# gopro/cineform-sdk

Hardware: AMD Instinct MI355X
Metric: 1080p YUY2 encode+decode fps (higher is better)
Workload: dtype int16

## Files before the change

cineform-sdk_amd/csrc/cfhd_entropy_gpu.h:

```cpp
#pragma once
#include "cfhd_core.h"
#include "cfhd_bitstream.h"
#include "cfhd_gop.h"
#include <vector>

namespace cfhd {

int device_stream_create(void **stream);
void device_stream_destroy(void *stream);
void device_stream_release(void *stream);
void device_streams_lean(bool on);
bool device_streams_are_lean();
struct StreamScope { StreamScope(); explicit StreamScope(void *preset ); ~StreamScope(); void *stream() const; };


class GpuEntropyEncoder {
public:
	GpuEntropyEncoder();
	~GpuEntropyEncoder();
	int prepare(const FramePlan &plan, int nframes, int16_t *d_coeffs, size_t coeff_stride_elems, size_t sample_cap, void *stream);
	int set_frame_header(int i, const SampleHeaderInfo &hdr);
	void set_plan(const FramePlan &plan) { plan_ = plan; }
	int prepare_group(const GopPlan &plan, int ngroups, int16_t *d_coeffs, size_t coeff_stride_elems, size_t sample_cap, void *stream);
	void set_group_plan(const GopPlan &plan) { gplan_ = plan; }
	int launch();
	int download();
	int download_queue();
	int download_finish();
	int fetch_sizes();
	const uint32_t *device_sizes() const { return d_sizes_; }
	const uint8_t *host_sample(int i) const { return h_samples_ + h_offsets_[i]; }
	uint8_t *device_sample(int i) { return d_samples_ + (size_t)i * cap_; }
	uint32_t sample_bytes(int i) const { return h_sizes_[i]; }
	void set_active(int k) { active_ = k; }
	void set_speculative_download(bool on) { speculative_download_ = on; if (!on) expect_bytes_ = 0; }
	bool needs_peak_table(int i) const { return peak_flags_in_use() && (h_sizes_[n_ + i] & 2u) != 0; }
	bool has_peak_table(int i) const { return peak_flags_in_use() && (h_sizes_[n_ + i] & 1u) != 0; }
	bool peak_flags_in_use() const { return group_ ? gplan_.interlaced : plan_.interlaced; }
	size_t sample_cap() const { return cap_; }
	int total_segments() const { return total_segs_; }
	float kernel_ms(int k);
	void set_level1_event(void *ev) { ev_level1_ = ev; }
	void *block_slots() const { return d_blocks_; }
	unsigned long long *block_masks(int frame) const { return d_masks_ ? d_masks_ + (size_t)frame * masks_per_frame_ : nullptr; }
	void set_block_lists(bool on) { use_blocks_ = on && d_blocks_; }
	bool block_lists() const { return use_blocks_; }
	void *headers_event() const { return ev_[3]; }
	void *samples_event() const { return ev_[4]; }
private:
	struct Host; Host *host_;
	void release();
	int prepare_units(int n, int16_t *d_coeffs, size_t coeff_stride_elems, size_t sample_cap, void *stream);
	void build_template(const SampleHeaderInfo &hdr, SampleTemplate *t) const;
	bool group_ = false; GopPlan gplan_;
	FramePlan plan_; int n_ = 0, active_ = 0, device_ = 0 ; size_t cap_ = 0; void *stream_ = nullptr;
	int active_frames() const { return active_ > 0 && active_ < n_ ? active_ : n_; }
	int nbands_ = 0, total_segs_ = 0;
	std::vector<SampleTemplate> tmpl_;
	uint8_t *d_samples_ = nullptr, *h_samples_ = nullptr;
	uint32_t *d_sizes_ = nullptr, *h_sizes_ = nullptr;
	uint8_t *d_packed_ = nullptr; uint32_t *d_offsets_ = nullptr, *h_offsets_ = nullptr;
	size_t expect_bytes_ = 0, copied_ahead_ = 0; int expect_frames_ = 0; bool speculative_download_ = false;
	void *d_tables_ = nullptr, *d_bands_ = nullptr, *d_segband_ = nullptr, *d_segs_ = nullptr, *d_bandstate_ = nullptr, *d_frames_ = nullptr, *d_tokens_ = nullptr;
	uint8_t *d_tmpl_ = nullptr, *h_tmpl_ = nullptr;
	bool dirty_ = true;
	void *ev_[5] = {nullptr, nullptr, nullptr, nullptr, nullptr}; bool timed_ = false;
	bool split_ = false, serial_split_ = false; void *ev_level1_ = nullptr, *stream2_ = nullptr, *ev2_[3] = {nullptr, nullptr, nullptr};
	int16_t *d_coeffs_ = nullptr; size_t coeff_stride_ = 0;
	void *d_blocks_ = nullptr; unsigned long long *d_masks_ = nullptr; size_t masks_per_frame_ = 0; bool use_blocks_ = false;
};


class GpuEntropyDecoder {
public:
	GpuEntropyDecoder();
	~GpuEntropyDecoder();
	void set_interlaced(bool on) { interlaced_ = on; }
	void set_active(int k) { active_ = k; }
	void set_skip_level1(bool skip) { skip_level1_ = skip; }
	int prepare(const FramePlan &plan, int nframes, int16_t *d_coeffs, size_t coeff_stride_elems, size_t sample_cap, int out_pixel_kind, void *stream);
	int set_sample_host(int i, const uint8_t *sample, size_t size);
	int set_sample_device(int i, const uint8_t *d_sample, const uint8_t *host_copy, size_t size);
	int set_samples_device(const uint8_t *d_samples, size_t stride_bytes, const uint32_t *d_sizes);
	void set_producer_events(void *headers, void *payloads) { ev_headers_ = headers; ev_payloads_ = payloads; }
	int launch();
	int check();
	float kernel_ms(int k);
	bool chunk_indexed() const { return dx_; }
	void *levels23_event() const { return l23_split_ ? ev_l23_ : nullptr; }
	void set_block_lists(bool on) { use_blocks_ = on && d_masks_; }
	bool level1_as_block_lists() const { return blocks_written_; }
	void dense_pyramid_uploaded() { blocks_written_ = false; }
	const unsigned long long *block_masks(int frame) const { return d_masks_ ? d_masks_ + (size_t)frame * masks_per_frame_ : nullptr; }
	int stats(uint32_t out[16]);
private:
	struct Host; Host *host_;
	void release();
	FramePlan plan_; int n_ = 0, out_kind_ = 0; size_t cap_ = 0, coeff_stride_ = 0; void *stream_ = nullptr;
	int16_t *d_coeffs_ = nullptr;
	uint8_t *d_samples_ = nullptr, *h_samples_ = nullptr;
	void *d_tables_ = nullptr, *d_bandjobs_ = nullptr, *d_lowjobs_ = nullptr, *d_plan_ = nullptr;
	void *ev_headers_ = nullptr, *ev_payloads_ = nullptr;
	bool skip_level1_ = false, interlaced_ = false; void *d_diffjobs_ = nullptr;
	int active_ = 0;
	int active_frames() const { return active_ > 0 && active_ < n_ ? active_ : n_; }
	const uint8_t *ext_samples_ = nullptr; size_t ext_stride_ = 0; const uint32_t *ext_sizes_ = nullptr;
	int *d_errors_ = nullptr, *h_errors_ = nullptr;
	bool lane_kernel_ = false;
	bool dx_ = true;
	void *d_tile_start_ = nullptr, *d_stats_ = nullptr, *d_repair_ = nullptr, *d_alts_ = nullptr, *d_reindex_ = nullptr, *d_alt_entries_ = nullptr; uint32_t alt_slots_ = 0;
	void *d_idx_tables_ = nullptr, *d_entries_ = nullptr, *d_recs_ = nullptr, *d_chunk_base_ = nullptr, *d_chunk_job_ = nullptr, *d_sums_ = nullptr, *d_counters_ = nullptr;
	uint32_t max_chunks_ = 0, *h_counters_ = nullptr; void *h_chunk_job_ = nullptr;
	int grid_index_ = 0, grid_tiles_ = 0;
	int device_ = 0;
	int launch_dx(bool device_jobs, int njobs, uint32_t host_chunks, int lowpass_jobs);
	void *ev_l23_ = nullptr, *ev_low_ = nullptr; bool l23_split_ = false;
	void *ev_[8] = {nullptr, nullptr, nullptr, nullptr, nullptr, nullptr, nullptr, nullptr}; bool timed_ = false;
	bool parse_end_ = false;
	unsigned long long *d_masks_ = nullptr; size_t masks_per_frame_ = 0; bool use_blocks_ = false, blocks_written_ = false;
};

class GpuGroupEntropyDecoder {
public:
	GpuGroupEntropyDecoder() {}
	~GpuGroupEntropyDecoder() { release(); }
	int prepare(const GopPlan &plan, int16_t *d_coeffs, size_t sample_cap, int out_pixel_kind, void *stream, int device = -1);
	int launch(const uint8_t *sample, size_t size, const ParsedGroup &pg);
	int check();
	void release();
private:
	GopPlan plan_; int out_kind_ = 0, device_ = 0; size_t cap_ = 0; void *stream_ = nullptr;
	int16_t *d_coeffs_ = nullptr;
	uint8_t *d_sample_ = nullptr, *h_sample_ = nullptr;
	void *d_tables_ = nullptr, *d_bandjobs_ = nullptr, *d_lowjobs_ = nullptr, *h_bandjobs_ = nullptr, *h_lowjobs_ = nullptr;
	void *d_tables18_ = nullptr, *d_diffjobs_ = nullptr, *h_diffjobs_ = nullptr;
	int *d_errors_ = nullptr, *h_errors_ = nullptr;
};

}
```

cineform-sdk_amd/csrc/cfhd_entropy_gpu.hip:

```cpp
#include "cfhd_entropy_gpu.h"
#include "cfhd_entropy_jobs.h"
#include <hip/hip_runtime.h>
#include <string.h>
#include <stdio.h>
#include <stdlib.h>
#include <algorithm>

namespace cfhd {

int device_init();
int device_current();
namespace { int g_fail(hipError_t e, const char *what) { fprintf(stderr, "[cfhd_amd] %s: %s\n", what, hipGetErrorString(e)); return (int)e ? (int)e : -1; } }
#define HIPCHK(expr) do { hipError_t _e = (expr); if (_e != hipSuccess) return g_fail(_e, #expr); } while (0)

struct GpuEntropyEncoder::Host { EntHostJobs jobs; std::vector<EntHoleGeom> geom; dev::EntFrameJob *frames = nullptr;  };

GpuEntropyEncoder::GpuEntropyEncoder() : host_(new Host) {}
GpuEntropyEncoder::~GpuEntropyEncoder() { release(); delete host_; }

void GpuEntropyEncoder::release()
{
	(void)hipSetDevice(device_);
	void *dev[] = { d_samples_, d_sizes_, d_tables_, d_bands_, d_segband_, d_segs_, d_bandstate_, d_frames_, d_tmpl_, d_packed_, d_offsets_, d_tokens_, d_blocks_, d_masks_ };
	for (void *p : dev) if (p) (void)hipFree(p);
	if (h_samples_) (void)hipHostFree(h_samples_);
	if (h_sizes_) (void)hipHostFree(h_sizes_);
	if (h_offsets_) (void)hipHostFree(h_offsets_);
	d_packed_ = nullptr; d_offsets_ = h_offsets_ = nullptr;
	if (h_tmpl_) (void)hipHostFree(h_tmpl_);
	if (host_->frames) { (void)hipHostFree(host_->frames); host_->frames = nullptr; }
	for (void *&e : ev_) if (e) { (void)hipEventDestroy((hipEvent_t)e); e = nullptr; }
	for (void *&e : ev2_) if (e) { (void)hipEventDestroy((hipEvent_t)e); e = nullptr; }
	if (stream2_) { device_stream_destroy(stream2_); stream2_ = nullptr; }
	timed_ = false;
	d_samples_ = h_samples_ = nullptr; d_sizes_ = h_sizes_ = nullptr; d_tables_ = d_bands_ = d_segband_ = d_segs_ = d_bandstate_ = d_frames_ = d_tokens_ = nullptr;
	d_tmpl_ = h_tmpl_ = nullptr; n_ = 0;
	d_blocks_ = nullptr; d_masks_ = nullptr; masks_per_frame_ = 0; use_blocks_ = false;
}

int GpuEntropyEncoder::prepare(const FramePlan &plan, int nframes, int16_t *d_coeffs, size_t stride, size_t sample_cap, void *stream)
{
	group_ = false; plan_ = plan;
	return prepare_units(nframes, d_coeffs, stride, sample_cap, stream);
}

int GpuEntropyEncoder::prepare_group(const GopPlan &plan, int ngroups, int16_t *d_coeffs, size_t stride, size_t sample_cap, void *stream)
{
	group_ = true; gplan_ = plan; plan_ = FramePlan(); plan_.interlaced = false;
	return prepare_units(ngroups, d_coeffs, stride, sample_cap, stream);
}

void GpuEntropyEncoder::build_template(const SampleHeaderInfo &hdr, SampleTemplate *t) const
{
	if (group_) build_group_template(gplan_, hdr, t); else build_sample_template(plan_, hdr, t);
}

int GpuEntropyEncoder::prepare_units(int nframes, int16_t *d_coeffs, size_t stride, size_t sample_cap, void *stream)
{
	int rc = device_init();
	if (rc) return rc;
	release();
	device_ = device_current(); (void)hipSetDevice(device_);
	const FramePlan &plan = plan_;
	n_ = nframes; cap_ = (sample_cap + 255) & ~(size_t)255; stream_ = stream; d_coeffs_ = d_coeffs; coeff_stride_ = stride;
	if (cap_ * (size_t)n_ >= ((size_t)1 << 32)) { fprintf(stderr, "[cfhd_amd] batch of %d frames exceeds the 4 GiB sample arena\n", n_); return -5; }
	{
		std::vector<dev::EntTables> h(2);
		ent_build_tables(&h[0], 1); ent_build_tables(&h[1], 2);
		HIPCHK(hipMalloc(&d_tables_, 2 * sizeof(dev::EntTables)));
		HIPCHK(hipMemcpy(d_tables_, h.data(), 2 * sizeof(dev::EntTables), hipMemcpyHostToDevice));
	}
	SampleHeaderInfo hdr0 = { 1, 2, 2, 4, !plan.interlaced, nullptr, 0, nullptr, 0 };
	tmpl_.assign(n_, SampleTemplate());
	build_template(hdr0, &tmpl_[0]);
	EntHostJobs &jobs = host_->jobs;
	host_->geom = group_ ? ent_hole_geometry(gplan_, tmpl_[0]) : ent_hole_geometry(plan, tmpl_[0]);
	if (!ent_build_band_jobs(host_->geom, tmpl_[0], n_, d_coeffs, stride, &jobs)) return -3;
	nbands_ = jobs.nbands; total_segs_ = (int)jobs.segjobs.size();
	HIPCHK(hipMalloc(&d_bands_, jobs.bands.size() * sizeof(dev::EntBandJob)));
	HIPCHK(hipMemcpy(d_bands_, jobs.bands.data(), jobs.bands.size() * sizeof(dev::EntBandJob), hipMemcpyHostToDevice));
	HIPCHK(hipMalloc(&d_segband_, jobs.segjobs.size() * sizeof(dev::EntSegJob)));
	HIPCHK(hipMemcpy(d_segband_, jobs.segjobs.data(), jobs.segjobs.size() * sizeof(dev::EntSegJob), hipMemcpyHostToDevice));
	HIPCHK(hipMalloc(&d_segs_, jobs.segjobs.size() * sizeof(dev::EntSegState)));
	HIPCHK(hipMalloc(&d_tokens_, jobs.segjobs.size() * (size_t)dev::ENT_TOK_STRIDE * sizeof(uint32_t)));
	HIPCHK(hipMalloc(&d_bandstate_, jobs.bands.size() * sizeof(dev::EntBandState)));
	static_assert((int)kBlockChunkCols == (int)dev::FWD_CHUNK_COLS_ENT, "one chunk geometry");
	if (!group_ && !plan.interlaced && plan.encoded_format == ENC_YUV422 && (plan.pixel_kind == PIX_YUY2 || plan.pixel_kind == PIX_2VUY) && plan.width % 32 == 0) {
		int mask_base[kMaxChannels][kNumBands];
		masks_per_frame_ = (size_t)block_list_layout(plan, mask_base);
		HIPCHK(hipMalloc(&d_blocks_, stride * 2 * (size_t)n_));
		HIPCHK(hipMalloc((void **)&d_masks_, masks_per_frame_ * 8 * (size_t)n_ + 64));
		HIPCHK(hipMemset(d_masks_, 0, masks_per_frame_ * 8 * (size_t)n_ + 64));
	}
	HIPCHK(hipMalloc((void **)&d_samples_, cap_ * n_));
	HIPCHK(hipHostMalloc((void **)&h_samples_, cap_ * n_, hipHostMallocPortable));
	HIPCHK(hipMalloc((void **)&d_sizes_, sizeof(uint32_t) * 2 * n_));
	HIPCHK(hipHostMalloc((void **)&h_sizes_, sizeof(uint32_t) * 2 * n_, hipHostMallocPortable));
	memset(h_sizes_, 0, sizeof(uint32_t) * 2 * n_);
	HIPCHK(hipMalloc((void **)&d_packed_, cap_ * n_));
	HIPCHK(hipMalloc((void **)&d_offsets_, sizeof(uint32_t) * (n_ + 1)));
	HIPCHK(hipHostMalloc((void **)&h_offsets_, sizeof(uint32_t) * (n_ + 1), hipHostMallocPortable));
	memset(h_offsets_, 0, sizeof(uint32_t) * (n_ + 1));
	HIPCHK(hipMalloc((void **)&d_tmpl_, (size_t)kEntTmplStride * n_));
	HIPCHK(hipHostMalloc((void **)&h_tmpl_, (size_t)kEntTmplStride * n_, hipHostMallocPortable));
	memset(h_tmpl_, 0, (size_t)kEntTmplStride * n_);
	HIPCHK(hipMalloc(&d_frames_, n_ * sizeof(dev::EntFrameJob)));
	HIPCHK(hipHostMalloc((void **)&host_->frames, n_ * sizeof(dev::EntFrameJob), hipHostMallocPortable));
	for (int f = 0; f < n_; f++) { SampleHeaderInfo h = hdr0; h.frame_number = (uint32_t)f + 1; if ((rc = set_frame_header(f, h))) return rc; }
	for (void *&e : ev_) HIPCHK(hipEventCreate((hipEvent_t *)&e));
	for (void *&e : ev2_) HIPCHK(hipEventCreate((hipEvent_t *)&e));
	if (n_ >= 8 || !device_streams_are_lean()) HIPCHK((hipError_t)device_stream_create(&stream2_));
	return 0;
}

int GpuEntropyEncoder::set_frame_header(int f, const SampleHeaderInfo &hdr)
{
	if (f < 0 || f >= n_) return -1;
	SampleTemplate &t = tmpl_[f];
	build_template(hdr, &t);
	if (!ent_fill_frame_block(host_->geom, t, f, host_->jobs, d_coeffs_ + (size_t)f * coeff_stride_, h_tmpl_ + (size_t)kEntTmplStride * f)) return -4;
	host_->frames[f] = ent_frame_job(t, d_tmpl_ + (size_t)kEntTmplStride * f, d_samples_ + cap_ * f, (uint32_t)cap_, d_sizes_ + f, d_sizes_ + n_ + f);
	dirty_ = true;
	return 0;
}

int GpuEntropyEncoder::launch()
{
	(void)hipSetDevice(device_);
	hipStream_t st = (hipStream_t)stream_;
	if (dirty_) {
		HIPCHK(hipMemcpyAsync(d_tmpl_, h_tmpl_, (size_t)kEntTmplStride * n_, hipMemcpyHostToDevice, st));
		HIPCHK(hipMemcpyAsync(d_frames_, host_->frames, n_ * sizeof(dev::EntFrameJob), hipMemcpyHostToDevice, st));
		dirty_ = false;
	}
	const dev::EntTables *T = (const dev::EntTables *)d_tables_;
	const dev::EntBatchGeom geom = { total_segs_ / n_, nbands_, coeff_stride_ };
	const int act = active_frames(), total_segs = total_segs_ / n_ * act;
	(void)hipGetLastError();
	HIPCHK(hipEventRecord((hipEvent_t)ev_[0], st));
#ifdef CFHD_AMD_PROBES
	const int count_probe = []{ const char *e = getenv("CFHD_AMD_COUNT_PROBE"); return e ? atoi(e) : 0; }();
#else
	const int count_probe = 0;
#endif
	const dev::EntBlockLists lists = { (const uint4 *)d_blocks_, d_masks_, d_coeffs_, masks_per_frame_ };
	auto count_range = [&](hipStream_t s, int lo, int n, bool level1 = false) {
		const int total = n * act;
		if (level1 && use_blocks_)
			dev::k_ent_count_blocks<<<(total + dev::ENT_WAVES - 1) / dev::ENT_WAVES, dev::ENT_THREADS, 0, s>>>((const dev::EntSegJob *)d_segband_, geom, total, (dev::EntSegState *)d_segs_, T,
			                                                                                                 d_sizes_ + n_, (uint32_t *)d_tokens_, lo, n, lists);
		else
			dev::k_ent_count<<<(total + dev::ENT_WAVES - 1) / dev::ENT_WAVES, dev::ENT_THREADS, 0, s>>>((const dev::EntSegJob *)d_segband_, geom, total, (dev::EntSegState *)d_segs_, T,
			                                                                                          d_sizes_ + n_, (uint32_t *)d_tokens_, lo, n, count_probe);
	};
	static const bool split_on = [] { const char *e = getenv("CFHD_AMD_COUNT_SPLIT"); return !(e && atoi(e) == 0); }();
	split_ = split_on && ev_level1_ && stream2_ && !host_->jobs.ranges_l1.empty() && act >= 8;
	if (peak_flags_in_use() && !split_) HIPCHK(hipMemsetAsync(d_sizes_ + n_, 0, sizeof(uint32_t) * n_, st));
	serial_split_ = split_ && stream2_ == stream_;
	if (serial_split_) {
		if (peak_flags_in_use()) HIPCHK(hipMemsetAsync(d_sizes_ + n_, 0, sizeof(uint32_t) * n_, st));
		HIPCHK(hipEventRecord((hipEvent_t)ev2_[0], st));
		for (const auto &r : host_->jobs.ranges_l1) count_range(st, r.first, r.second, true);
		HIPCHK(hipEventRecord((hipEvent_t)ev2_[1], st));
		for (const auto &r : host_->jobs.ranges_rest) count_range(st, r.first, r.second);
		HIPCHK(hipEventRecord((hipEvent_t)ev2_[2], st));
	} else if (split_) {
		hipStream_t s2 = (hipStream_t)stream2_;
		HIPCHK(hipStreamWaitEvent(s2, (hipEvent_t)ev_level1_, 0));
		if (peak_flags_in_use()) HIPCHK(hipMemsetAsync(d_sizes_ + n_, 0, sizeof(uint32_t) * n_, s2));
		HIPCHK(hipEventRecord((hipEvent_t)ev2_[0], s2));
		for (const auto &r : host_->jobs.ranges_l1) count_range(s2, r.first, r.second, true);
		HIPCHK(hipEventRecord((hipEvent_t)ev2_[1], s2));
		for (const auto &r : host_->jobs.ranges_rest) count_range(st, r.first, r.second);
		HIPCHK(hipEventRecord((hipEvent_t)ev2_[2], st));
		HIPCHK(hipStreamWaitEvent(st, (hipEvent_t)ev2_[1], 0));
	} else if (use_blocks_) {
		for (const auto &r : host_->jobs.ranges_l1) count_range(st, r.first, r.second, true);
		for (const auto &r : host_->jobs.ranges_rest) count_range(st, r.first, r.second);
	} else count_range(st, 0, total_segs_ / n_);
	HIPCHK(hipEventRecord((hipEvent_t)ev_[1], st));
	dev::k_ent_scan<<<nbands_ * act, dev::ENT_THREADS, 0, st>>>((const dev::EntBandJob *)d_bands_, (dev::EntSegState *)d_segs_, (dev::EntBandState *)d_bandstate_, T);
	HIPCHK(hipEventRecord((hipEvent_t)ev_[2], st));
	const unsigned layout_parts = act >= 256 ? 8u : (unsigned)((2048 + act - 1) / act > 256 ? 256 : (2048 + act - 1) / act);
	dev::k_ent_layout<<<dim3((unsigned)act, layout_parts), dev::ENT_THREADS, 0, st>>>((const dev::EntFrameJob *)d_frames_, (const dev::EntBandJob *)d_bands_, (dev::EntSegState *)d_segs_,
	                                                  (dev::EntBandState *)d_bandstate_, T);
	HIPCHK(hipEventRecord((hipEvent_t)ev_[3], st));
	{
		dev::EntPeakHoles which; which.n = 0;
		for (size_t h = 0; h < tmpl_[0].holes.size() && which.n < 7; h++) if (tmpl_[0].holes[h].kind == 2) which.hole[which.n++] = (int)h;
		if (which.n) dev::k_ent_peaks<<<dim3(act >= 64 ? 4u : 32u, (unsigned)which.n, (unsigned)act), dev::ENT_THREADS, 0, st>>>((const dev::EntFrameJob *)d_frames_, which, (const dev::EntBandJob *)d_bands_,
		                                                  (const dev::EntSegJob *)d_segband_, geom, (const dev::EntSegState *)d_segs_, (const dev::EntBandState *)d_bandstate_);
	}
#ifdef CFHD_AMD_PROBES
	const int emit_probe = []{ const char *e = getenv("CFHD_AMD_EMIT_PROBE"); return e ? atoi(e) : 0; }();
#else
	const int emit_probe = 0;
#endif
	dev::k_ent_emit<<<(total_segs + dev::ENT_WAVES * dev::ENT_EMIT_SEGS - 1) / (dev::ENT_WAVES * dev::ENT_EMIT_SEGS), dev::ENT_THREADS, 0, st>>>(total_segs, (const dev::EntSegState *)d_segs_,
	                                                          T, (const uint32_t *)d_tokens_, emit_probe);
	HIPCHK(hipGetLastError());
	HIPCHK(hipEventRecord((hipEvent_t)ev_[4], st));
	timed_ = true;
	return 0;
}

float GpuEntropyEncoder::kernel_ms(int k)
{
	float ms = 0;
	if (!timed_ || k < 0 || k > 4) return 0;
	if (k == 4) {
		if (!split_ || hipEventElapsedTime(&ms, (hipEvent_t)ev2_[0], (hipEvent_t)ev2_[1]) != hipSuccess) { (void)hipGetLastError(); return 0; }
		return ms;
	}
	void *end = (k == 0 && split_) ? ev2_[2] : ev_[k + 1];
	void *begin = (k == 0 && serial_split_) ? ev2_[1] : ev_[k];
	if (hipEventElapsedTime(&ms, (hipEvent_t)begin, (hipEvent_t)end) != hipSuccess) { (void)hipGetLastError(); return 0; }
	return ms;
}

int GpuEntropyEncoder::fetch_sizes()
{
	(void)hipSetDevice(device_);
	hipStream_t st = (hipStream_t)stream_;
	HIPCHK(hipMemcpyAsync(h_sizes_, d_sizes_, sizeof(uint32_t) * 2 * n_, hipMemcpyDeviceToHost, st));
	HIPCHK(hipStreamSynchronize(st));
	return 0;
}

int GpuEntropyEncoder::download() { const int rc = download_queue(); return rc ? rc : download_finish(); }

int GpuEntropyEncoder::download_queue()
{
	(void)hipSetDevice(device_);
	hipStream_t st = (hipStream_t)stream_;
	const bool direct = false;
	(void)hipGetLastError();
	const int act = active_frames();
	dev::k_ent_pack_offsets<<<1, dev::ENT_THREADS, 0, st>>>(d_sizes_, act, d_offsets_);
	dev::k_ent_pack<<<dim3(direct ? 2 : 8, (unsigned)act), dev::ENT_THREADS, 0, st>>>(d_samples_, cap_, d_sizes_, d_offsets_, direct ? h_samples_ : d_packed_);
	HIPCHK(hipGetLastError());
	HIPCHK(hipMemcpyAsync(h_sizes_, d_sizes_, sizeof(uint32_t) * 2 * n_, hipMemcpyDeviceToHost, st));
	HIPCHK(hipMemcpyAsync(h_offsets_, d_offsets_, sizeof(uint32_t) * (act + 1), hipMemcpyDeviceToHost, st));
	copied_ahead_ = 0;
	if (!direct && expect_bytes_ && expect_frames_ == act) {
		copied_ahead_ = expect_bytes_ < cap_ * (size_t)act ? expect_bytes_ : cap_ * (size_t)act;
		HIPCHK(hipMemcpyAsync(h_samples_, d_packed_, copied_ahead_, hipMemcpyDeviceToHost, st));
	}
	return 0;
}

int GpuEntropyEncoder::download_finish()
{
	(void)hipSetDevice(device_);
	hipStream_t st = (hipStream_t)stream_;
	const bool direct = false;
	const int act = active_frames();
	HIPCHK(hipStreamSynchronize(st));
	const size_t total = h_offsets_[act];
	if (!direct && total > copied_ahead_) HIPCHK(hipMemcpyAsync(h_samples_ + copied_ahead_, d_packed_ + copied_ahead_, total - copied_ahead_, hipMemcpyDeviceToHost, st));
	expect_bytes_ = speculative_download_ ? ((total + total / 32 + 4095) & ~(size_t)4095) : 0; expect_frames_ = act;
	return 0;
}

struct GpuEntropyDecoder::Host {
	std::vector<std::vector<dev::DecBandJob>> bands;
	std::vector<std::vector<dev::DecLowpassJob>> lows;
	std::vector<size_t> host_bytes;
	std::vector<std::vector<dev::DecDiffJob>> diffs;
	dev::DecBandJob *flat_bands = nullptr; dev::DecLowpassJob *flat_lows = nullptr; dev::DecDiffJob *flat_diffs = nullptr;
};

GpuEntropyDecoder::GpuEntropyDecoder() : host_(new Host) {}
GpuEntropyDecoder::~GpuEntropyDecoder() { release(); delete host_; }

void GpuEntropyDecoder::release()
{
	(void)hipSetDevice(device_);
	void *dev[] = { d_samples_, d_tables_, d_bandjobs_, d_lowjobs_, d_errors_, d_plan_, d_idx_tables_, d_entries_, d_recs_, d_chunk_base_, d_chunk_job_, d_sums_, d_counters_, d_tile_start_, d_stats_, d_repair_, d_alts_, d_reindex_, d_diffjobs_, d_alt_entries_, d_masks_ };
	d_masks_ = nullptr; masks_per_frame_ = 0; use_blocks_ = false; blocks_written_ = false;
	for (void *p : dev) if (p) (void)hipFree(p);
	d_idx_tables_ = d_entries_ = d_recs_ = d_chunk_base_ = d_chunk_job_ = d_sums_ = d_counters_ = d_tile_start_ = d_stats_ = d_repair_ = d_alts_ = d_reindex_ = d_diffjobs_ = d_alt_entries_ = nullptr;
	if (h_chunk_job_) (void)hipHostFree(h_chunk_job_);
	if (h_counters_) (void)hipHostFree(h_counters_);
	h_chunk_job_ = nullptr; h_counters_ = nullptr;
	if (h_samples_) (void)hipHostFree(h_samples_);
	if (h_errors_) (void)hipHostFree(h_errors_);
	if (host_->flat_bands) { (void)hipHostFree(host_->flat_bands); host_->flat_bands = nullptr; }
	if (host_->flat_lows) { (void)hipHostFree(host_->flat_lows); host_->flat_lows = nullptr; }
	if (host_->flat_diffs) { (void)hipHostFree(host_->flat_diffs); host_->flat_diffs = nullptr; }
	for (void *&e : ev_) if (e) { (void)hipEventDestroy((hipEvent_t)e); e = nullptr; }
	if (ev_l23_) { (void)hipEventDestroy((hipEvent_t)ev_l23_); ev_l23_ = nullptr; }
	if (ev_low_) { (void)hipEventDestroy((hipEvent_t)ev_low_); ev_low_ = nullptr; }
	timed_ = false;
	d_samples_ = h_samples_ = nullptr; d_tables_ = d_bandjobs_ = d_lowjobs_ = d_plan_ = nullptr; d_errors_ = h_errors_ = nullptr; n_ = 0; ext_samples_ = nullptr;
}

int GpuEntropyDecoder::prepare(const FramePlan &plan, int nframes, int16_t *d_coeffs, size_t stride, size_t sample_cap, int out_kind, void *stream)
{
	int rc = device_init();
	if (rc) return rc;
	release();
	device_ = device_current(); (void)hipSetDevice(device_);
	plan_ = plan; n_ = nframes; cap_ = (sample_cap + 255) & ~(size_t)255; stream_ = stream; d_coeffs_ = d_coeffs; coeff_stride_ = stride; out_kind_ = out_kind;
	std::vector<uint32_t> t = build_dec_tables(1);
	HIPCHK(hipMalloc(&d_tables_, t.size() * 4));
	HIPCHK(hipMemcpy(d_tables_, t.data(), t.size() * 4, hipMemcpyHostToDevice));
	HIPCHK(hipMalloc((void **)&d_samples_, cap_ * n_));
	HIPCHK(hipHostMalloc((void **)&h_samples_, cap_ * n_, hipHostMallocPortable));
	const size_t max_bands = (size_t)n_ * kMaxChannels * 9, max_lows = (size_t)n_ * kMaxChannels;
	HIPCHK(hipMalloc(&d_bandjobs_, max_bands * sizeof(dev::DecBandJob)));
	HIPCHK(hipMalloc(&d_lowjobs_, max_lows * sizeof(dev::DecLowpassJob)));
	HIPCHK(hipHostMalloc((void **)&host_->flat_bands, max_bands * sizeof(dev::DecBandJob), hipHostMallocPortable));
	HIPCHK(hipHostMalloc((void **)&host_->flat_lows, max_lows * sizeof(dev::DecLowpassJob), hipHostMallocPortable));
	HIPCHK(hipMalloc(&d_diffjobs_, max_lows * sizeof(dev::DecDiffJob)));
	HIPCHK(hipHostMalloc((void **)&host_->flat_diffs, max_lows * sizeof(dev::DecDiffJob), hipHostMallocPortable));
	HIPCHK(hipMalloc((void **)&d_errors_, sizeof(int)));
	HIPCHK(hipHostMalloc((void **)&h_errors_, sizeof(int), hipHostMallocPortable));
	*h_errors_ = 0;
	{ const char *e = getenv("CFHD_AMD_DEC"); lane_kernel_ = e && strcmp(e, "lane") == 0; dx_ = !(e && (strcmp(e, "lane") == 0 || strcmp(e, "par") == 0)); }
	if (dx_) {
		dev::DecIdxTables *it = new dev::DecIdxTables;
		const bool ok = build_dec_index_tables(1, it);
		if (ok) { hipError_t e = hipMalloc(&d_idx_tables_, sizeof(*it)); if (e == hipSuccess) e = hipMemcpy(d_idx_tables_, it, sizeof(*it), hipMemcpyHostToDevice); if (e != hipSuccess) { delete it; return g_fail(e, "decoder tables"); } }
		delete it;
		if (!ok) return -6;
		const size_t per_frame = cap_ / dev::DX_CHUNK_BYTES + (size_t)kMaxChannels * 9 + 1;
		if (per_frame * (size_t)n_ >= ((size_t)1 << 31) / dev::DX_ENTRY_STRIDE * 8) return -5;
		max_chunks_ = (uint32_t)(per_frame * (size_t)n_);
		HIPCHK(hipMalloc(&d_entries_, (size_t)max_chunks_ * dev::DX_ENTRY_STRIDE * 4));
		HIPCHK(hipMalloc(&d_recs_, (size_t)max_chunks_ * sizeof(dev::DxChunkRec)));
		HIPCHK(hipMalloc(&d_chunk_base_, (size_t)max_chunks_ * 4));
		HIPCHK(hipMalloc(&d_chunk_job_, (size_t)max_chunks_ * sizeof(dev::DxChunkDesc)));
		HIPCHK(hipMalloc(&d_sums_, max_bands * sizeof(dev::DxBandSum)));
		HIPCHK(hipMalloc(&d_counters_, 32));
		HIPCHK(hipMalloc(&d_repair_, max_bands * 4));
		HIPCHK(hipMalloc(&d_alts_, (size_t)max_chunks_ * sizeof(dev::DxChunkAlt)));
		HIPCHK(hipMalloc(&d_reindex_, (size_t)max_chunks_ * sizeof(dev::DxReindex)));
		alt_slots_ = max_chunks_ / 8 > 64u ? max_chunks_ / 8 : 64u;
		HIPCHK(hipMalloc(&d_alt_entries_, (size_t)alt_slots_ * dev::DX_ENTRY_STRIDE * 4));
		{
			dev::DecPlan dp0; dec_build_plan(plan, out_kind, &dp0);
			const dev::DxTilePlan tp0 = dx_tile_plan(plan, dp0, n_, false);
			HIPCHK(hipMalloc(&d_tile_start_, ((size_t)tp0.total + 1) * sizeof(dev::DxTileDesc)));
			const char *se = getenv("CFHD_AMD_DX_STATS");
			if (se && atoi(se)) { HIPCHK(hipMalloc(&d_stats_, 64)); HIPCHK(hipMemset(d_stats_, 0, 64)); }
		}
		HIPCHK(hipHostMalloc((void **)&h_chunk_job_, (size_t)max_chunks_ * sizeof(dev::DxChunkDesc), hipHostMallocPortable));
		HIPCHK(hipHostMalloc((void **)&h_counters_, 32, hipHostMallocPortable));
		int cus = 256;
		(void)hipDeviceGetAttribute(&cus, hipDeviceAttributeMultiprocessorCount, device_current());
		grid_index_ = cus * 5; grid_tiles_ = cus * (int)((160 * 1024) / (sizeof(uint2) * (1 << dev::DX_KM) + sizeof(uint32_t) * (dev::DX_LONG11_MAX + dev::DX_TILE_WORDS)));
		if (const char *e = getenv("CFHD_AMD_DX_GRID_TILES")) if (atoi(e) > 0) grid_tiles_ = atoi(e);
		if (grid_index_ < 1) grid_index_ = 1;
		if (grid_tiles_ < 1) grid_tiles_ = 1;
	}
	{
		dev::DecPlan dp;
		dec_build_plan(plan, out_kind, &dp);
		HIPCHK(hipMalloc(&d_plan_, sizeof(dp)));
		HIPCHK(hipMemcpy(d_plan_, &dp, sizeof(dp), hipMemcpyHostToDevice));
	}
	if (dx_ && plan.encoded_format == ENC_YUV422 && plan.num_channels == 3) {
		int mask_base[kMaxChannels][kNumBands];
		masks_per_frame_ = (size_t)dec_block_list_layout(plan, mask_base);
		HIPCHK(hipMalloc((void **)&d_masks_, masks_per_frame_ * 8 * (size_t)n_));
	}
	host_->bands.assign(n_, {}); host_->lows.assign(n_, {}); host_->diffs.assign(n_, {}); host_->host_bytes.assign(n_, 0);
	for (void *&e : ev_) HIPCHK(hipEventCreate((hipEvent_t *)&e));
	HIPCHK(hipEventCreate((hipEvent_t *)&ev_l23_));
	HIPCHK(hipEventCreate((hipEvent_t *)&ev_low_));
	return 0;
}

int GpuEntropyDecoder::set_samples_device(const uint8_t *d_samples, size_t stride_bytes, const uint32_t *d_sizes)
{
	if (!d_samples || !d_sizes || (stride_bytes & 255) || ((uintptr_t)d_samples & 255)) return -1;
	ext_samples_ = d_samples; ext_stride_ = stride_bytes; ext_sizes_ = d_sizes;
	return 0;
}

int GpuEntropyDecoder::set_sample_host(int i, const uint8_t *sample, size_t size)
{
	if (i < 0 || i >= n_ || size > cap_) return -1;
	memcpy(h_samples_ + cap_ * i, sample, size);
	int rc = set_sample_device(i, d_samples_ + cap_ * i, sample, size);
	if (rc == 0) host_->host_bytes[i] = (size + 3) & ~(size_t)3;
	return rc;
}

int GpuEntropyDecoder::set_sample_device(int i, const uint8_t *d_sample, const uint8_t *host_copy, size_t size)
{
	if (i < 0 || i >= n_) return -1;
	ext_samples_ = nullptr;
	ParsedSample ps;
	if (parse_sample(host_copy, size, &ps) != 0) return -2;
	if (ps.width != plan_.width || ps.display_height != plan_.display_height || ps.encoded_format != plan_.encoded_format || ps.num_channels != plan_.num_channels) return -3;
	host_->bands[i].clear(); host_->lows[i].clear(); host_->host_bytes[i] = 0;
	if (dx_) {
		dev::DecPlan dp; dec_build_plan(plan_, out_kind_, &dp);
		host_->bands[i].assign((size_t)dp.bands_per_frame, dev::DecBandJob());
		host_->lows[i].assign((size_t)plan_.num_channels, dev::DecLowpassJob());
		host_->diffs[i].assign((size_t)plan_.num_channels, dev::DecDiffJob());
		if (!dx_build_jobs(ps, plan_, dp, d_sample, d_coeffs_ + (size_t)i * coeff_stride_, out_kind_, 0, 1, host_->bands[i].data(), host_->lows[i].data(), skip_level1_,
		                   interlaced_ ? host_->diffs[i].data() : nullptr)) return -4;
		return 0;
	}
	if (interlaced_) return -4;
	if (!dec_build_jobs(ps, plan_, d_sample, d_coeffs_ + (size_t)i * coeff_stride_, out_kind_, &host_->bands[i], &host_->lows[i], skip_level1_)) return -4;
	return 0;
}

enum { kLowLatencyFrames = 32 };

int GpuEntropyDecoder::launch()
{
	(void)hipSetDevice(device_);
	hipStream_t st = (hipStream_t)stream_;
	l23_split_ = false; blocks_written_ = false;
	if (ext_samples_) {
		const int nch = plan_.num_channels, nb = n_ * nch * 9;
		HIPCHK(hipMemsetAsync(d_errors_, 0, sizeof(int), st));
		(void)hipGetLastError();
		static const bool parse_early = [] { const char *e = getenv("CFHD_AMD_PARSE_EARLY"); return !(e && atoi(e) == 0); }();
		if (!parse_early && ev_payloads_) ev_headers_ = ev_payloads_;
		if (ev_headers_) HIPCHK(hipStreamWaitEvent(st, (hipEvent_t)ev_headers_, 0));
		HIPCHK(hipEventRecord((hipEvent_t)ev_[0], st));
		dev::k_dec_parse<<<n_, dev::DEC_PARSE_THREADS, 0, st>>>(ext_samples_, ext_stride_, ext_sizes_, n_,
			(const dev::DecPlan *)d_plan_, d_coeffs_, coeff_stride_, (dev::DecBandJob *)d_bandjobs_, (dev::DecLowpassJob *)d_lowjobs_, d_errors_,
			interlaced_ && dx_ ? (dev::DecDiffJob *)d_diffjobs_ : nullptr);
		parse_end_ = ev_payloads_ != nullptr;
		if (parse_end_) { HIPCHK(hipEventRecord((hipEvent_t)ev_[4], st)); HIPCHK(hipStreamWaitEvent(st, (hipEvent_t)ev_payloads_, 0)); }
		ev_headers_ = ev_payloads_ = nullptr;
		HIPCHK(hipEventRecord((hipEvent_t)ev_[1], st));
		l23_split_ = false;
		if (dx_) { const int rc_dx = launch_dx(true, nb, 0u, n_ * nch); if (rc_dx) return rc_dx; }
		else if (n_ <= kLowLatencyFrames) dev::k_dec_bands_par_ll<<<nb, dev::DECP_LL_THREADS, 0, st>>>((const dev::DecBandJob *)d_bandjobs_, (const dev::DecTables *)d_tables_, d_errors_);
		else dev::k_dec_bands_par<<<nb, dev::DECP_THREADS, 0, st>>>((const dev::DecBandJob *)d_bandjobs_, (const dev::DecTables *)d_tables_, d_errors_);
		HIPCHK(hipEventRecord((hipEvent_t)ev_[2], st));
		if (!l23_split_) dev::k_dec_lowpass<<<dim3(8, (unsigned)(n_ * nch)), 256, 0, st>>>((const dev::DecLowpassJob *)d_lowjobs_);
		HIPCHK(hipGetLastError());
		HIPCHK(hipEventRecord((hipEvent_t)ev_[3], st));
		timed_ = true;
		HIPCHK(hipMemcpyAsync(h_errors_, d_errors_, sizeof(int), hipMemcpyDeviceToHost, st));
		return 0;
	}
	parse_end_ = false;
	if (dx_) {
		dev::DecPlan dp; dec_build_plan(plan_, out_kind_, &dp);
		const int nch = plan_.num_channels, act = active_frames(), nb = dp.bands_per_frame * act;
		HIPCHK(hipStreamSynchronize(st));
		for (int f = 0; f < act; f++) {
			if ((int)host_->bands[f].size() != dp.bands_per_frame || (int)host_->lows[f].size() != nch) return -1;
			for (int s = 0; s < dp.bands_per_frame; s++) host_->flat_bands[(size_t)s * act + f] = host_->bands[f][s];
			for (int c = 0; c < nch; c++) host_->flat_lows[(size_t)f * nch + c] = host_->lows[f][c];
			if (interlaced_) { if ((int)host_->diffs[f].size() != nch) return -1; for (int c = 0; c < nch; c++) host_->flat_diffs[(size_t)f * nch + c] = host_->diffs[f][c]; }
		}
		std::vector<dev::DxChunkDesc> cj;
		const uint32_t nchunks = dx_number_chunks(host_->flat_bands, nb, &cj);
		if (nchunks > max_chunks_) return -5;
		memcpy(h_chunk_job_, cj.data(), cj.size() * sizeof(dev::DxChunkDesc));
		h_counters_[0] = nchunks; h_counters_[1] = 0; h_counters_[2] = 0; h_counters_[3] = 0; h_counters_[4] = 0;
		HIPCHK(hipMemsetAsync(d_errors_, 0, sizeof(int), st));
		for (int f = 0; f < act; f++)
			if (host_->host_bytes[f]) HIPCHK(hipMemcpyAsync(d_samples_ + cap_ * f, h_samples_ + cap_ * f, host_->host_bytes[f], hipMemcpyHostToDevice, st));
		HIPCHK(hipMemcpyAsync(d_bandjobs_, host_->flat_bands, (size_t)nb * sizeof(dev::DecBandJob), hipMemcpyHostToDevice, st));
		HIPCHK(hipMemcpyAsync(d_lowjobs_, host_->flat_lows, (size_t)act * nch * sizeof(dev::DecLowpassJob), hipMemcpyHostToDevice, st));
		if (interlaced_) HIPCHK(hipMemcpyAsync(d_diffjobs_, host_->flat_diffs, (size_t)act * nch * sizeof(dev::DecDiffJob), hipMemcpyHostToDevice, st));
		HIPCHK(hipMemcpyAsync(d_chunk_job_, h_chunk_job_, (size_t)nchunks * sizeof(dev::DxChunkDesc), hipMemcpyHostToDevice, st));
		HIPCHK(hipMemcpyAsync(d_counters_, h_counters_, 20, hipMemcpyHostToDevice, st));
		(void)hipGetLastError();
		HIPCHK(hipEventRecord((hipEvent_t)ev_[0], st));
		HIPCHK(hipEventRecord((hipEvent_t)ev_[1], st));
		l23_split_ = false;
		int rc = launch_dx(false, nb, nchunks, act * nch);
		if (rc) return rc;
		HIPCHK(hipEventRecord((hipEvent_t)ev_[2], st));
		if (!l23_split_) dev::k_dec_lowpass<<<dim3(8, (unsigned)(act * nch)), 256, 0, st>>>((const dev::DecLowpassJob *)d_lowjobs_);
		HIPCHK(hipGetLastError());
		HIPCHK(hipEventRecord((hipEvent_t)ev_[3], st));
		timed_ = true;
		HIPCHK(hipMemcpyAsync(h_errors_, d_errors_, sizeof(int), hipMemcpyDeviceToHost, st));
		return 0;
	}
	const bool lane_kernel = lane_kernel_;
	dev::DecBandJob *fb = host_->flat_bands; dev::DecLowpassJob *fl = host_->flat_lows;
	size_t nfb = 0, nfl = 0, per_frame = 0;
	for (int f = 0; f < n_; f++) per_frame = host_->bands[f].size() > per_frame ? host_->bands[f].size() : per_frame;
	for (size_t k = 0; k < per_frame; k++) for (int f = 0; f < n_; f++) if (k < host_->bands[f].size()) fb[nfb++] = host_->bands[f][k];
	for (int f = 0; f < n_; f++) for (const dev::DecLowpassJob &j : host_->lows[f]) fl[nfl++] = j;
	if (!nfb) return -1;
	if (!lane_kernel) std::stable_sort(fb, fb + nfb, [](const dev::DecBandJob &a, const dev::DecBandJob &b) { return a.bytes > b.bytes; });
	else HIPCHK(hipMemset2DAsync(d_coeffs_, coeff_stride_ * 2, 0, (size_t)plan_.final_elems * 2, n_, st));
	HIPCHK(hipMemsetAsync(d_errors_, 0, sizeof(int), st));
	for (int f = 0; f < n_; f++)
		if (host_->host_bytes[f]) HIPCHK(hipMemcpyAsync(d_samples_ + cap_ * f, h_samples_ + cap_ * f, host_->host_bytes[f], hipMemcpyHostToDevice, st));
	HIPCHK(hipMemcpyAsync(d_bandjobs_, fb, nfb * sizeof(dev::DecBandJob), hipMemcpyHostToDevice, st));
	HIPCHK(hipMemcpyAsync(d_lowjobs_, fl, nfl * sizeof(dev::DecLowpassJob), hipMemcpyHostToDevice, st));
	(void)hipGetLastError();
	const int nb = (int)nfb;
	HIPCHK(hipEventRecord((hipEvent_t)ev_[0], st));
	HIPCHK(hipEventRecord((hipEvent_t)ev_[1], st));
	if (lane_kernel) dev::k_dec_bands<<<(nb + dev::DEC_THREADS - 1) / dev::DEC_THREADS, dev::DEC_THREADS, 0, st>>>((const dev::DecBandJob *)d_bandjobs_, nb, (const dev::DecTables *)d_tables_, d_errors_);
	else if (n_ <= kLowLatencyFrames) dev::k_dec_bands_par_ll<<<nb, dev::DECP_LL_THREADS, 0, st>>>((const dev::DecBandJob *)d_bandjobs_, (const dev::DecTables *)d_tables_, d_errors_);
	else dev::k_dec_bands_par<<<nb, dev::DECP_THREADS, 0, st>>>((const dev::DecBandJob *)d_bandjobs_, (const dev::DecTables *)d_tables_, d_errors_);
	HIPCHK(hipEventRecord((hipEvent_t)ev_[2], st));
	dev::k_dec_lowpass<<<dim3(8, (unsigned)nfl), 256, 0, st>>>((const dev::DecLowpassJob *)d_lowjobs_);
	HIPCHK(hipGetLastError());
	HIPCHK(hipEventRecord((hipEvent_t)ev_[3], st));
	timed_ = true;
	HIPCHK(hipMemcpyAsync(h_errors_, d_errors_, sizeof(int), hipMemcpyDeviceToHost, st));
	return 0;
}

int GpuEntropyDecoder::launch_dx(bool device_jobs, int njobs, uint32_t host_chunks, int lowpass_jobs)
{
	hipStream_t st = (hipStream_t)stream_;
	dev::DecBandJob *jobs = (dev::DecBandJob *)d_bandjobs_;
	const dev::DecIdxTables *T = (const dev::DecIdxTables *)d_idx_tables_;
	dev::DecPlan dp; dec_build_plan(plan_, out_kind_, &dp);
	const int frames = device_jobs ? n_ : active_frames();
	const bool lists = use_blocks_ && d_masks_ && !skip_level1_;
	const dev::DxTilePlan tp = dx_tile_plan(plan_, dp, frames, skip_level1_, lists, interlaced_);
	unsigned long long *const tmasks = lists ? d_masks_ : nullptr;
	blocks_written_ = lists;
	const char *spec_env = getenv("CFHD_AMD_DX_SPECULATE");
	const bool speculate = !(spec_env && atoi(spec_env) == 0);
	if (device_jobs) HIPCHK(hipMemsetAsync((uint32_t *)d_counters_ + 1, 0, 16, st));
	if (device_jobs) {
		dev::k_dec_plan<<<1, 1024, 0, st>>>(jobs, njobs, max_chunks_, (uint32_t *)d_counters_, d_errors_);
		dev::k_dec_plan_fill<<<(njobs + dev::DX_WAVES - 1) / dev::DX_WAVES, dev::DX_THREADS, 0, st>>>(jobs, njobs, (dev::DxChunkDesc *)d_chunk_job_, (const uint32_t *)d_counters_);
	}
	HIPCHK(hipEventRecord((hipEvent_t)ev_[7], st));
	const uint32_t chunk_bound = device_jobs ? max_chunks_ : host_chunks;
	int g1 = grid_index_, g3 = grid_tiles_;
	if ((uint32_t)g1 * dev::DX_WAVES > chunk_bound) g1 = (int)((chunk_bound + dev::DX_WAVES - 1) / dev::DX_WAVES);
	const uint32_t tile_waves = 1u;
	if ((uint32_t)g3 > tp.total) g3 = (int)tp.total;
	if (g1 < 1) g1 = 1;
	if (g3 < 1) g3 = 1;
	dev::k_dec_index<<<g1, dev::DX_THREADS, 0, st>>>((const dev::DxChunkDesc *)d_chunk_job_, (const uint32_t *)d_counters_, T, (uint32_t *)d_entries_, (dev::DxChunkRec *)d_recs_, (dev::DxChunkAlt *)d_alts_, speculate ? 1 : 0, (uint32_t *)d_stats_,
	                                                 (uint32_t *)d_alt_entries_, alt_slots_, (uint32_t *)d_counters_ + 3, (uint32_t *)d_counters_ + 4);
	HIPCHK(hipEventRecord((hipEvent_t)ev_[5], st));
	dev::k_dec_chain<<<(njobs + dev::DX_WAVES - 1) / dev::DX_WAVES, dev::DX_THREADS, 0, st>>>(jobs, njobs, (const dev::DxChunkRec *)d_recs_, (const dev::DxChunkAlt *)d_alts_, (uint32_t *)d_chunk_base_,
	                                                                                            (dev::DxBandSum *)d_sums_, d_errors_, (uint32_t *)d_repair_, (dev::DxReindex *)d_reindex_, (uint32_t *)d_counters_);
	const int small_grid = njobs < 256 ? (njobs + dev::DX_WAVES - 1) / dev::DX_WAVES : 64;
	dev::k_dec_repair<<<small_grid, dev::DX_THREADS, 0, st>>>(jobs, T, (uint32_t *)d_entries_, (dev::DxChunkRec *)d_recs_, (const dev::DxChunkAlt *)d_alts_, (uint32_t *)d_chunk_base_, (dev::DxBandSum *)d_sums_,
	                                                         d_errors_, (const uint32_t *)d_repair_, (dev::DxReindex *)d_reindex_, (uint32_t *)d_counters_, (uint32_t *)d_stats_);
	dev::k_dec_reindex<<<g1, dev::DX_THREADS, 0, st>>>(jobs, T, (uint32_t *)d_entries_, (const dev::DxReindex *)d_reindex_, (const uint32_t *)d_counters_, (uint32_t *)d_stats_,
	                                                   (const dev::DxChunkAlt *)d_alts_, (const uint32_t *)d_alt_entries_);
	dev::k_dec_tile_index<<<(tp.total + dev::DX_TILE_INDEX_TILES - 1) / dev::DX_TILE_INDEX_TILES, dev::DX_THREADS, 0, st>>>(jobs, tp, (const uint32_t *)d_entries_, (const uint32_t *)d_chunk_base_, (const dev::DxBandSum *)d_sums_,
	                                                                                                  (dev::DxTileDesc *)d_tile_start_, tmasks, (uint32_t)masks_per_frame_);
	HIPCHK(hipEventRecord((hipEvent_t)ev_[6], st));
	const char *split_env = getenv("CFHD_AMD_TILES_SPLIT");
	l23_split_ = frames >= 8 && !skip_level1_ && tp.split > 0 && tp.split < tp.total && split_env && split_env[0] == '1';
	auto tile_pass = [&](const dev::DxTilePlan &p, int g) {
		dev::k_dec_tiles<dev::DX_TILE_THREADS><<<g < 1 ? 1 : g, dev::DX_TILE_THREADS, 0, st>>>((const dev::DxTileDesc *)d_tile_start_, p.first, p.total, T, (const uint32_t *)d_entries_, (const uint32_t *)d_chunk_base_);
	};
	if (l23_split_) {
		dev::DxTilePlan ta = tp, tb = tp;
		ta.total = tp.split; tb.first = tp.split;
		int ga = g3, gb = g3;
		if ((uint32_t)ga * tile_waves > ta.total) ga = (int)((ta.total + tile_waves - 1) / tile_waves);
		if ((uint32_t)gb * tile_waves > tb.total - tb.first) gb = (int)((tb.total - tb.first + tile_waves - 1) / tile_waves);
		tile_pass(ta, ga);
		HIPCHK(hipEventRecord((hipEvent_t)ev_low_, st));
		dev::k_dec_lowpass<<<dim3(8, (unsigned)lowpass_jobs), 256, 0, st>>>((const dev::DecLowpassJob *)d_lowjobs_);
		HIPCHK(hipEventRecord((hipEvent_t)ev_l23_, st));
		tile_pass(tb, gb);
	} else tile_pass(tp, g3);
	if (interlaced_) {
		const bool rows = true;
		if (rows) dev::k_dec_undiff_rows<<<dim3((unsigned)(frames * plan_.num_channels), 32), 64 * dev::DXR_WAVES, 0, st>>>((const dev::DecDiffJob *)d_diffjobs_);
		dev::k_dec_undiff<<<dim3((unsigned)(frames * plan_.num_channels), dev::DXU_SPLIT), dev::DXU_THREADS, 0, st>>>((const dev::DecDiffJob *)d_diffjobs_, d_errors_, rows ? 1 : 0);
	}
	HIPCHK(hipGetLastError());
	return 0;
}

int GpuEntropyDecoder::check() { return *h_errors_ ? -1 : 0; }

int GpuEntropyDecoder::stats(uint32_t out[16])
{
	(void)hipSetDevice(device_);
	memset(out, 0, 64);
	if (!d_stats_) return -1;
	HIPCHK(hipStreamSynchronize((hipStream_t)stream_));
	HIPCHK(hipMemcpy(out, d_stats_, 64, hipMemcpyDeviceToHost));
	return 0;
}

float GpuEntropyDecoder::kernel_ms(int k)
{
	float ms = 0;
	if (k >= 3) {
		if (!timed_ || !dx_ || k > 6) return 0;
		void *a = k == 3 ? ev_[7] : (k == 4 ? ev_[5] : (k == 5 ? ev_[6] : ev_[1])), *b = k == 3 ? ev_[5] : (k == 4 ? ev_[6] : (k == 5 ? ev_[2] : ev_[7]));
		if (hipEventElapsedTime(&ms, (hipEvent_t)a, (hipEvent_t)b) != hipSuccess) { (void)hipGetLastError(); return 0; }
		if (k == 5 && l23_split_) {
			float low = 0;
			if (hipEventElapsedTime(&low, (hipEvent_t)ev_low_, (hipEvent_t)ev_l23_) == hipSuccess) ms -= low; else (void)hipGetLastError();
		}
		return ms;
	}
	if (k == 2 && l23_split_ && timed_) {
		if (hipEventElapsedTime(&ms, (hipEvent_t)ev_low_, (hipEvent_t)ev_l23_) != hipSuccess) { (void)hipGetLastError(); return 0; }
		return ms;
	}
	void *end = (k == 0 && parse_end_) ? ev_[4] : ev_[k + 1];
	if (!timed_ || k < 0 || k > 2 || hipEventElapsedTime(&ms, (hipEvent_t)ev_[k], (hipEvent_t)end) != hipSuccess) { (void)hipGetLastError(); return 0; }
	return ms;
}

void GpuGroupEntropyDecoder::release()
{
	(void)hipSetDevice(device_);
	void *dev[] = { d_sample_, d_tables_, d_tables18_, d_bandjobs_, d_lowjobs_, d_diffjobs_, d_errors_ };
	for (void *p : dev) if (p) (void)hipFree(p);
	void *host[] = { h_sample_, h_bandjobs_, h_lowjobs_, h_diffjobs_, h_errors_ };
	for (void *p : host) if (p) (void)hipHostFree(p);
	d_sample_ = h_sample_ = nullptr; d_tables_ = d_tables18_ = d_bandjobs_ = d_lowjobs_ = d_diffjobs_ = h_bandjobs_ = h_lowjobs_ = h_diffjobs_ = nullptr; d_errors_ = h_errors_ = nullptr;
}

enum { kGroupBandJobs = 3 * 15, kGroupRawJobs = 3 * 2, kGroupDiffJobs = 3 * 2 };

int GpuGroupEntropyDecoder::prepare(const GopPlan &plan, int16_t *d_coeffs, size_t sample_cap, int out_kind, void *stream, int device)
{
	int rc = device_init();
	if (rc) return rc;
	release();
	device_ = device >= 0 ? device : device_current(); (void)hipSetDevice(device_);
	plan_ = plan; d_coeffs_ = d_coeffs; cap_ = (sample_cap + 255) & ~(size_t)255; out_kind_ = out_kind; stream_ = stream;
	std::vector<uint32_t> t = build_dec_tables(1);
	HIPCHK(hipMalloc(&d_tables_, t.size() * 4));
	HIPCHK(hipMemcpy(d_tables_, t.data(), t.size() * 4, hipMemcpyHostToDevice));
	t = build_dec_tables(2);
	HIPCHK(hipMalloc(&d_tables18_, t.size() * 4));
	HIPCHK(hipMemcpy(d_tables18_, t.data(), t.size() * 4, hipMemcpyHostToDevice));
	HIPCHK(hipMalloc(&d_diffjobs_, kGroupDiffJobs * sizeof(dev::DecDiffJob)));
	HIPCHK(hipHostMalloc(&h_diffjobs_, kGroupDiffJobs * sizeof(dev::DecDiffJob), hipHostMallocPortable));
	HIPCHK(hipMalloc((void **)&d_sample_, cap_));
	HIPCHK(hipHostMalloc((void **)&h_sample_, cap_, hipHostMallocPortable));
	HIPCHK(hipMalloc(&d_bandjobs_, kGroupBandJobs * sizeof(dev::DecBandJob)));
	HIPCHK(hipMalloc(&d_lowjobs_, kGroupRawJobs * sizeof(dev::DecLowpassJob)));
	HIPCHK(hipHostMalloc(&h_bandjobs_, kGroupBandJobs * sizeof(dev::DecBandJob), hipHostMallocPortable));
	HIPCHK(hipHostMalloc(&h_lowjobs_, kGroupRawJobs * sizeof(dev::DecLowpassJob), hipHostMallocPortable));
	HIPCHK(hipMalloc((void **)&d_errors_, sizeof(int)));
	HIPCHK(hipHostMalloc((void **)&h_errors_, sizeof(int), hipHostMallocPortable));
	*h_errors_ = 0;
	return 0;
}

int GpuGroupEntropyDecoder::launch(const uint8_t *sample, size_t size, const ParsedGroup &pg)
{
	(void)hipSetDevice(device_);
	hipStream_t st = (hipStream_t)stream_;
	if (size > cap_) return -1;
	HIPCHK(hipStreamSynchronize(st));
	dev::DecBandJob *bj = (dev::DecBandJob *)h_bandjobs_; dev::DecLowpassJob *lj = (dev::DecLowpassJob *)h_lowjobs_; dev::DecDiffJob *dj = (dev::DecDiffJob *)h_diffjobs_;
	int nb = 0, nl = 0, nd = 0;
	for (int c = 0; c < 3; c++) {
		const GopChannel &ch = plan_.ch[c];
		const ParsedBand &lp = pg.lowpass[c];
		const GopWavelet &top = ch.w[5];
		if (!lp.present || lp.width != top.width || lp.height != top.height || (size_t)lp.offset + (size_t)top.width * top.height * 2 > size) return -2;
		lj[nl++] = dev::DecLowpassJob{ d_sample_ + lp.offset, d_coeffs_ + top.offset[0], top.width, top.height, top.pitch, 2 * lowpass_bias(10, top.width, out_kind_) };
		static const int coded[5] = { 5, 4, 3, 1, 0 };
		for (int k : coded) {
			const GopWavelet &wv = ch.w[k];
			for (int b = (k == 3 ? 0 : 1); b < 4; b++) {
				const ParsedBand &pb = pg.band[c][k][b];
				if (!pb.present || pb.width != wv.width || pb.height != wv.height || (pb.offset & 3) || (size_t)pb.offset + pb.bytes > size) return -2;
				if (pb.codebook < 0) {
					if ((size_t)pb.bytes < (size_t)wv.width * wv.height * 2 || pb.quant != 1 || (wv.width & 1)) return -3;
					lj[nl++] = dev::DecLowpassJob{ d_sample_ + pb.offset, d_coeffs_ + wv.offset[0], wv.width, wv.height, wv.pitch, 0 };
					continue;
				}
				const bool diff = gop_band_is_difference_coded(plan_, k, b);
				if (pb.codebook != (diff ? 2 : 1) || pb.difference != diff || (wv.offset[b] & 7) || (wv.pitch & 7)) return -3;
				if (diff) {
					if (nd >= kGroupDiffJobs || wv.width > 16 * 256 || (pb.peak_level && (size_t)pb.peak_offset + 2 > size)) return -3;
					dj[nd++] = dev::DecDiffJob{ d_coeffs_ + wv.offset[b], wv.width, wv.height, wv.pitch, pb.peak_level ? d_sample_ + pb.peak_offset : nullptr,
					                            pb.peak_level ? (uint32_t)(size - pb.peak_offset) : 0u, pb.peak_level };
				}
				bj[nb++] = dev::DecBandJob{ d_sample_ + pb.offset, pb.bytes, d_coeffs_ + wv.offset[b], wv.height * wv.pitch, pb.quant, 0u, diff ? 1 : 0 };
			}
		}
	}
	if (nb != kGroupBandJobs || nl != kGroupRawJobs || nd != (plan_.interlaced ? kGroupDiffJobs : 0)) return -2;
	std::stable_sort(bj, bj + nb, [](const dev::DecBandJob &a, const dev::DecBandJob &b) { return a.table != b.table ? a.table < b.table : a.bytes > b.bytes; });
	const int nb18 = nd, nb17 = nb - nb18;
	memcpy(h_sample_, sample, size);
	HIPCHK(hipMemsetAsync(d_errors_, 0, sizeof(int), st));
	HIPCHK(hipMemcpyAsync(d_sample_, h_sample_, (size + 3) & ~(size_t)3, hipMemcpyHostToDevice, st));
	HIPCHK(hipMemcpyAsync(d_bandjobs_, bj, nb * sizeof(dev::DecBandJob), hipMemcpyHostToDevice, st));
	HIPCHK(hipMemcpyAsync(d_lowjobs_, lj, nl * sizeof(dev::DecLowpassJob), hipMemcpyHostToDevice, st));
	(void)hipGetLastError();
	dev::k_dec_bands_par_ll<<<nb17, dev::DECP_LL_THREADS, 0, st>>>((const dev::DecBandJob *)d_bandjobs_, (const dev::DecTables *)d_tables_, d_errors_);
	if (nb18) {
		HIPCHK(hipMemcpyAsync(d_diffjobs_, dj, nd * sizeof(dev::DecDiffJob), hipMemcpyHostToDevice, st));
		dev::k_dec_bands_par_ll<<<nb18, dev::DECP_LL_THREADS, 0, st>>>((const dev::DecBandJob *)d_bandjobs_ + nb17, (const dev::DecTables *)d_tables18_, d_errors_);
		dev::k_dec_undiff<<<dim3((unsigned)nd, dev::DXU_SPLIT), dev::DXU_THREADS, 0, st>>>((const dev::DecDiffJob *)d_diffjobs_, d_errors_, 0);
	}
	dev::k_dec_lowpass<<<dim3(8, (unsigned)nl), 256, 0, st>>>((const dev::DecLowpassJob *)d_lowjobs_);
	HIPCHK(hipGetLastError());
	HIPCHK(hipMemcpyAsync(h_errors_, d_errors_, sizeof(int), hipMemcpyDeviceToHost, st));
	return 0;
}

int GpuGroupEntropyDecoder::check() { return h_errors_ ? *h_errors_ : -1; }

}
```

cineform-sdk_amd/csrc/cfhd_entropy_jobs.h:

```cpp
#pragma once
#include "cfhd_core.h"
#include "cfhd_bitstream.h"
#include "cfhd_gop.h"
#include "cfhd_entropy_kernels.h"
#include "cfhd_dec_kernels.h"
#include <vector>
#include <algorithm>
#include <string.h>

namespace cfhd {

enum { kEntTmplBytes = 6144, kEntWordHolesBytes = 1536, kEntHolesBytes = dev::ENT_MAX_HOLES * (int)sizeof(dev::EntHole), kEntMaxPatches = 96,
       kEntPatchBytes = kEntMaxPatches * (int)sizeof(dev::EntPatch), kEntTmplStride = kEntTmplBytes + kEntWordHolesBytes + kEntHolesBytes + kEntPatchBytes };

inline void ent_build_tables(dev::EntTables *h, int codebook = 1)
{
	const EntropyTables *t = entropy_tables(codebook);
	memcpy(h->value_code, t->value_code, sizeof(h->value_code));
	memcpy(h->run_bits, t->run_bits, sizeof(h->run_bits));
	for (int c = 0; c < 3072; c++) { h->run_count[c] = t->run_count[c]; h->run_size[c] = t->run_size[c]; }
	h->run_total[0] = 0;
	for (int c = 1; c < 3072; c++) h->run_total[c] = (uint16_t)(t->run_size[c] + h->run_total[c - t->run_count[c]]);
	h->band_end_bits = t->band_end_bits; h->band_end_size = t->band_end_size;
	for (int c = 0; c < 3072; c++) { h->run_pack[c].x = t->run_bits[c]; h->run_pack[c].y = (uint32_t)t->run_size[c] | ((uint32_t)t->run_count[c] << 8); }
}

std::vector<uint32_t> build_dec_tables(int codebook);

inline bool build_dec_index_tables(int codebook, dev::DecIdxTables *T)
{
	using namespace dev;
	memset(T, 0, sizeof(*T));
	RawCode codes[300];
	const int ncodes = raw_codes(codebook, codes);
	const EntropyTables *et = entropy_tables(codebook);
	for (int m = 0; m < 256; m++) { T->mag_expand[0][m] = entropy_tables(1)->mag_expand[m]; T->mag_expand[1][m] = entropy_tables(2)->mag_expand[m]; }
	(void)et;
	auto type_of = [](const RawCode &c) { return c.kind == 0 ? DX_T_RUN : (c.kind == 1 ? DX_T_VALUE : DX_T_END); };
	uint32_t nlong = 0;
	int l2_of_prefix[1 << DX_K];
	for (int p = 0; p < (1 << DX_K); p++) l2_of_prefix[p] = -1;
	for (int i = 0; i < ncodes; i++) {
		const RawCode &c = codes[i];
		if (c.len <= DX_K) {
			if (c.kind == 2 || c.payload >= (1 << 11) || c.len > 12) return false;
			const uint32_t base = c.bits << (DX_K - c.len);
			const uint16_t e = (uint16_t)(c.len | (c.kind == 1 ? 16 : 0) | (c.payload << 5));
			for (uint32_t k = 0; k < (1u << (DX_K - c.len)); k++) T->sym12[base + k] = e;
		} else {
			if (c.len > DX_K + 2 * DX_L2_BITS) return false;
			const uint32_t p = c.bits >> (c.len - DX_K);
			if (l2_of_prefix[p] < 0) {
				if (nlong + (1u << DX_L2_BITS) > DX_LONG_MAX || nlong >= (1u << 11)) return false;
				l2_of_prefix[p] = (int)nlong; nlong += 1u << DX_L2_BITS;
				T->sym12[p] = (uint16_t)(16u | ((uint32_t)l2_of_prefix[p] << 5));
			}
		}
	}
	struct L3 { uint32_t key; int maxlen; uint32_t base; };
	std::vector<L3> l3;
	for (int i = 0; i < ncodes; i++) {
		const RawCode &c = codes[i];
		if (c.len <= DX_K + DX_L2_BITS) continue;
		const uint32_t key = c.bits >> (c.len - DX_K - DX_L2_BITS);
		auto it = std::find_if(l3.begin(), l3.end(), [&](const L3 &x) { return x.key == key; });
		if (it == l3.end()) l3.push_back(L3{ key, c.len, 0 }); else if (c.len > it->maxlen) it->maxlen = c.len;
	}
	for (L3 &x : l3) {
		const int nb = x.maxlen - DX_K - DX_L2_BITS;
		if (nlong + (1u << nb) > DX_LONG_MAX) return false;
		x.base = nlong; nlong += 1u << nb;
		const uint32_t p = x.key >> DX_L2_BITS;
		T->long_tab[(uint32_t)l2_of_prefix[p] + (x.key & ((1u << DX_L2_BITS) - 1u))] = (uint32_t)nb | ((uint32_t)DX_T_ESCAPE << 5) | (x.base << 8);
	}
	for (int i = 0; i < ncodes; i++) {
		const RawCode &c = codes[i];
		if (c.len <= DX_K) continue;
		const uint32_t entry = (c.kind == 2 ? 0u : (uint32_t)c.len + (c.kind == 1 ? 1u : 0u)) | ((uint32_t)type_of(c) << 5) | ((c.kind == 0 ? (uint32_t)c.payload : (c.kind == 1 ? 1u : 0u)) << 8);
		if (c.len <= DX_K + DX_L2_BITS) {
			const uint32_t p = c.bits >> (c.len - DX_K);
			const int spare = DX_K + DX_L2_BITS - c.len;
			const uint32_t base = (uint32_t)l2_of_prefix[p] + ((c.bits & ((1u << (c.len - DX_K)) - 1u)) << spare);
			for (uint32_t k = 0; k < (1u << spare); k++) T->long_tab[base + k] = entry;
		} else {
			const uint32_t key = c.bits >> (c.len - DX_K - DX_L2_BITS);
			const L3 &x = *std::find_if(l3.begin(), l3.end(), [&](const L3 &y) { return y.key == key; });
			const int nb = x.maxlen - DX_K - DX_L2_BITS, rest = c.len - DX_K - DX_L2_BITS, spare = nb - rest;
			const uint32_t base = x.base + ((c.bits & ((1u << rest) - 1u)) << spare);
			for (uint32_t k = 0; k < (1u << spare); k++) T->long_tab[base + k] = entry;
		}
	}
	T->nlong = nlong;
	for (uint32_t win = 0; win < (1u << DX_K); win++) {
		int used = 0; uint32_t count = 0;
		for (;;) {
			const uint32_t rest = (win << used) & ((1u << DX_K) - 1u);
			const uint16_t e = T->sym12[rest];
			const int len = e & 15, total = len + ((e & 16) ? 1 : 0);
			if (!len || total > DX_K - used) break;
			const uint32_t add = (e & 16) ? 1u : (uint32_t)(e >> 5);
			if (count + add > 4095u) break;
			used += total; count += add;
		}
		T->cnt12[win] = (uint16_t)(used | (count << 4));
	}
	for (uint32_t win = 0; win < (1u << DX_KM); win++) {
		int used = 0, pre = 0, mid = 0, post = 0, v1 = 0, v2 = 0;
		for (;;) {
			const uint32_t rest = ((win << (DX_K - DX_KM)) << used) & ((1u << DX_K) - 1u);
			const uint16_t e = T->sym12[rest];
			const int len = e & 15, total = len + ((e & 16) ? 1 : 0);
			if (!len || total > DX_KM - used) break;
			if (e & 16) {
				if (v2) break;
				const int m = e >> 5;
				if (T->mag_expand[0][m] != m || T->mag_expand[1][m] != m || m > 0x7fff) return false;
				const int negative = (int)((rest >> (DX_K - len - 1)) & 1u);
				if (!v1) v1 = negative ? -m : m; else v2 = negative ? -m : m;
			} else {
				const int run = e >> 5;
				int *slot = v2 ? &post : (v1 ? &mid : &pre);
				if (*slot + run > (slot == &pre ? 0xfff : 0xff)) break;
				*slot += run;
			}
			used += total;
		}
		if (v1 && !v2) { post = mid; mid = 0; }
		const int total = pre + (v1 ? 1 : 0) + mid + (v2 ? 1 : 0) + post;
		const uint32_t o1 = v1 ? (uint32_t)pre : (uint32_t)DX_NO_VALUE, o2 = v2 ? (uint32_t)(pre + 1 + mid) : (uint32_t)DX_NO_VALUE;
		if (total > 0xfff || v1 < -128 || v1 > 127 || v2 < -128 || v2 > 127 || (v1 && pre >= (int)DX_NO_VALUE) || (v2 && pre + 1 + mid >= (int)DX_NO_VALUE)) return false;
		T->multi[win].x = (uint32_t)(used & 15) | ((uint32_t)total << 4) | (o1 << 16);
		T->multi[win].y = o2 | ((uint32_t)(uint8_t)(int8_t)v1 << 16) | ((uint32_t)(uint8_t)(int8_t)v2 << 24);
	}
	{
		auto entry_of = [&](const RawCode &c, bool *ok) {
			const uint32_t a = c.kind == 1 ? T->mag_expand[0][c.payload] : (c.kind == 0 ? (uint32_t)c.payload : 0u), b = c.kind == 1 ? T->mag_expand[1][c.payload] : a;
			const uint32_t bits = (uint32_t)c.len + (c.kind == 1 ? 1u : 0u);
			if (a >= (1u << 12) || b >= (1u << 12) || bits > 31u) *ok = false;
			return bits | ((uint32_t)type_of(c) << 5) | (a << 8) | (b << 20);
		};
		bool ok = true;
		uint32_t n11 = 0;
		int l2_of[1 << DX_KM];
		for (int p = 0; p < (1 << DX_KM); p++) l2_of[p] = -1;
		struct L3b { uint32_t key; int maxlen; uint32_t base; };
		std::vector<L3b> l3b;
		for (int i = 0; i < ncodes; i++) {
			const RawCode &c = codes[i];
			const int total = c.len + (c.kind == 1 ? 1 : 0);
			if (total <= DX_KM) continue;
			if (c.len <= DX_KM) {
				const uint32_t base = c.bits << (DX_KM - c.len);
				for (uint32_t k = 0; k < (1u << (DX_KM - c.len)); k++) { if (T->multi[base + k].x & 15u) ok = false; T->multi[base + k].y = entry_of(c, &ok); }
				continue;
			}
			const uint32_t p11 = c.bits >> (c.len - DX_KM);
			if (l2_of[p11] < 0) {
				if (n11 + (1u << DX_L11_BITS) > DX_LONG11_MAX) return false;
				l2_of[p11] = (int)n11; n11 += 1u << DX_L11_BITS;
				if (T->multi[p11].x & 15u) ok = false;
				T->multi[p11].y = (uint32_t)DX_L11_BITS | ((uint32_t)DX_T_ESCAPE << 5) | ((uint32_t)l2_of[p11] << 8);
			}
			if (c.len > DX_KM + DX_L11_BITS) {
				const uint32_t key = c.bits >> (c.len - DX_KM - DX_L11_BITS);
				auto it = std::find_if(l3b.begin(), l3b.end(), [&](const L3b &x) { return x.key == key; });
				if (it == l3b.end()) l3b.push_back(L3b{ key, c.len, 0 }); else if (c.len > it->maxlen) it->maxlen = c.len;
			}
		}
		for (L3b &x : l3b) {
			const int nb = x.maxlen - DX_KM - DX_L11_BITS;
			if (n11 + (1u << nb) > DX_LONG11_MAX) return false;
			x.base = n11; n11 += 1u << nb;
			T->long11[(uint32_t)l2_of[x.key >> DX_L11_BITS] + (x.key & ((1u << DX_L11_BITS) - 1u))] = (uint32_t)nb | ((uint32_t)DX_T_ESCAPE << 5) | (x.base << 8);
		}
		for (int i = 0; i < ncodes; i++) {
			const RawCode &c = codes[i];
			if (c.len <= DX_KM) continue;
			const uint32_t e = entry_of(c, &ok);
			if (c.len <= DX_KM + DX_L11_BITS) {
				const int spare = DX_KM + DX_L11_BITS - c.len;
				const uint32_t base = (uint32_t)l2_of[c.bits >> (c.len - DX_KM)] + ((c.bits & ((1u << (c.len - DX_KM)) - 1u)) << spare);
				for (uint32_t k = 0; k < (1u << spare); k++) T->long11[base + k] = e;
			} else {
				const uint32_t key = c.bits >> (c.len - DX_KM - DX_L11_BITS);
				const L3b &x = *std::find_if(l3b.begin(), l3b.end(), [&](const L3b &y) { return y.key == key; });
				const int nb = x.maxlen - DX_KM - DX_L11_BITS, rest = c.len - DX_KM - DX_L11_BITS, spare = nb - rest;
				const uint32_t base = x.base + ((c.bits & ((1u << rest) - 1u)) << spare);
				for (uint32_t k = 0; k < (1u << spare); k++) T->long11[base + k] = e;
			}
		}
		if (!ok) return false;
		for (uint32_t win = 0; win < (1u << DX_KM); win++) if ((T->multi[win].x & 15u) == 0 && (T->multi[win].x & 0xffffu)) return false;
	}
	return true;
}

struct EntHostJobs {
	std::vector<dev::EntBandJob> bands;
	std::vector<dev::EntSegJob> segjobs;
	std::vector<int> band_of_hole;
	int nbands = 0;
	std::vector<std::pair<int, int>> ranges_l1, ranges_rest;
};

struct EntHoleGeom { size_t offset; int width, height, pitch; int table ; int mask_base ; bool level1; };
inline std::vector<EntHoleGeom> ent_hole_geometry(const FramePlan &plan, const SampleTemplate &t)
{
	int mask_base[kMaxChannels][kNumBands];
	block_list_layout(plan, mask_base);
	std::vector<EntHoleGeom> g;
	for (const SampleTemplate::Hole &hole : t.holes) {
		const BandDesc &bd = plan.ch[hole.channel].band[hole.level][hole.band];
		g.push_back(EntHoleGeom{ bd.offset, bd.width, bd.height, bd.pitch,
		                         plan.interlaced && hole.level == 0 && hole.band == 2 ? 1 : 0,
		                         hole.kind == 1 && hole.level == 0 ? mask_base[hole.channel][hole.band] : -1, hole.level == 0 });
	}
	return g;
}
inline std::vector<EntHoleGeom> ent_hole_geometry(const GopPlan &plan, const SampleTemplate &t)
{
	std::vector<EntHoleGeom> g;
	for (const SampleTemplate::Hole &hole : t.holes) {
		const GopWavelet &wv = plan.ch[hole.channel].w[hole.level];
		g.push_back(EntHoleGeom{ wv.offset[hole.band], wv.width, wv.height, wv.pitch, gop_band_is_difference_coded(plan, hole.level, hole.band) ? 1 : 0, -1, hole.level < 2 });
	}
	return g;
}

inline bool ent_build_band_jobs(const std::vector<EntHoleGeom> &geom, const SampleTemplate &t0, int nframes, int16_t *coeffs, size_t stride, EntHostJobs *out)
{
	if ((int)t0.holes.size() > dev::ENT_MAX_HOLES || (int)t0.patches.size() > kEntMaxPatches || geom.size() != t0.holes.size()) return false;
	out->bands.clear(); out->segjobs.clear(); out->ranges_l1.clear(); out->ranges_rest.clear();
	out->band_of_hole.assign(t0.holes.size(), -1);
	for (int f = 0; f < nframes; f++) {
		int16_t *base = coeffs + (size_t)f * stride;
		for (size_t h = 0; h < t0.holes.size(); h++) {
			const SampleTemplate::Hole &hole = t0.holes[h];
			if (hole.kind != 1) continue;
			const EntHoleGeom &bd = geom[h];
			dev::EntBandJob j;
			j.coeffs = base + bd.offset; j.n = bd.height * bd.pitch;
			j.nseg = (j.n + dev::ENT_SEG - 1) / dev::ENT_SEG; j.seg_base = (int)out->segjobs.size();
			j.frame = f; j.hole = (int)h;
			j.table = bd.table;
			if (f == 0) {
				out->band_of_hole[h] = (int)out->bands.size();
				std::vector<std::pair<int, int>> &r = bd.level1 ? out->ranges_l1 : out->ranges_rest;
				if (!r.empty() && r.back().first + r.back().second == j.seg_base) r.back().second += j.nseg; else r.push_back({ j.seg_base, j.nseg });
			}
			for (int s = 0; s < j.nseg; s++) out->segjobs.push_back(dev::EntSegJob{ j.coeffs, j.n, s * dev::ENT_SEG, (int)out->bands.size(), j.table, bd.pitch, bd.mask_base });
			out->bands.push_back(j);
		}
	}
	out->nbands = (int)out->bands.size() / nframes;
	return true;
}
inline bool ent_build_band_jobs(const FramePlan &plan, const SampleTemplate &t0, int nframes, int16_t *coeffs, size_t stride, EntHostJobs *out)
{
	return ent_build_band_jobs(ent_hole_geometry(plan, t0), t0, nframes, coeffs, stride, out);
}

inline bool ent_fill_frame_block(const std::vector<EntHoleGeom> &geom, const SampleTemplate &t, int f, const EntHostJobs &jobs, const int16_t *coeffs_f, uint8_t *block)
{
	if (t.bytes.size() > (size_t)kEntTmplBytes || t.bytes.size() / 4 > (size_t)kEntWordHolesBytes || t.holes.size() != jobs.band_of_hole.size() ||
	    t.patches.size() > (size_t)kEntMaxPatches || geom.size() != t.holes.size()) return false;
	memcpy(block, t.bytes.data(), t.bytes.size());
	uint8_t *wh = block + kEntTmplBytes;
	size_t hole = 0;
	for (size_t w = 0; w < t.bytes.size() / 4; w++) {
		while (hole < t.holes.size() && (size_t)t.holes[hole].tmpl_offset <= w * 4) hole++;
		wh[w] = (uint8_t)hole;
	}
	dev::EntHole *eh = (dev::EntHole *)(block + kEntTmplBytes + kEntWordHolesBytes);
	for (size_t i = 0; i < t.holes.size(); i++) {
		const SampleTemplate::Hole &src = t.holes[i];
		const EntHoleGeom &bd = geom[i];
		dev::EntHole &d = eh[i];
		d.tmpl_offset = src.tmpl_offset; d.kind = src.kind; d.fixed_bytes = src.fixed_bytes;
		d.band_job = src.kind == 1 ? jobs.band_of_hole[i] + f * jobs.nbands : (src.kind == 2 && i > 0 && t.holes[i - 1].kind == 1 ? jobs.band_of_hole[i - 1] + f * jobs.nbands : -1);
		if (src.kind == 2 && d.band_job < 0) return false;
		d.lowpass = src.kind == 0 ? coeffs_f + bd.offset : nullptr;
		d.lp_width = bd.width; d.lp_height = bd.height; d.lp_pitch = bd.pitch;
	}
	dev::EntPatch *ep = (dev::EntPatch *)(block + kEntTmplBytes + kEntWordHolesBytes + kEntHolesBytes);
	for (size_t i = 0; i < t.patches.size(); i++) {
		const SampleTemplate::Patch &p = t.patches[i];
		ep[i].kind = p.kind; ep[i].at_tmpl = p.at_tmpl; ep[i].at_holes = p.at_holes; ep[i].start_tmpl = p.start_tmpl; ep[i].start_holes = p.start_holes;
		ep[i].end_tmpl = p.end_tmpl; ep[i].end_holes = p.end_holes; ep[i].tag = p.tag;
	}
	return true;
}
inline bool ent_fill_frame_block(const FramePlan &plan, const SampleTemplate &t, int f, const EntHostJobs &jobs, const int16_t *coeffs_f, uint8_t *block)
{
	return ent_fill_frame_block(ent_hole_geometry(plan, t), t, f, jobs, coeffs_f, block);
}

inline dev::EntFrameJob ent_frame_job(const SampleTemplate &t, uint8_t *block_addr, uint8_t *out, uint32_t out_cap, uint32_t *size_out, uint32_t *peak_flag)
{
	dev::EntFrameJob fj;
	fj.out = out; fj.out_cap = out_cap;
	fj.tmpl = block_addr; fj.tmpl_bytes = (int)t.bytes.size();
	fj.word_holes = block_addr + kEntTmplBytes;
	fj.holes = (const dev::EntHole *)(block_addr + kEntTmplBytes + kEntWordHolesBytes); fj.nholes = (int)t.holes.size();
	fj.patches = (const dev::EntPatch *)(block_addr + kEntTmplBytes + kEntWordHolesBytes + kEntHolesBytes); fj.npatches = (int)t.patches.size();
	fj.sample_bytes = size_out; fj.peak_flag = peak_flag;
	return fj;
}


inline bool dec_build_jobs(const ParsedSample &ps, const FramePlan &plan, const uint8_t *sample_addr, int16_t *coeff_base, int out_pixel_kind,
                           std::vector<dev::DecBandJob> *bands, std::vector<dev::DecLowpassJob> *lowpass, bool skip_level1 = false)
{
	for (int c = 0; c < plan.num_channels; c++) {
		const ParsedBand &lp = ps.lowpass[c];
		const BandDesc &ll = plan.ch[c].band[2][0];
		if (!lp.present || lp.width != ll.width || lp.height != ll.height) return false;
		dev::DecLowpassJob lj = { sample_addr + lp.offset, coeff_base + ll.offset, ll.width, ll.height, ll.pitch, lowpass_bias(plan.precision, ll.width, out_pixel_kind, c) };
		lowpass->push_back(lj);
		for (int lv = skip_level1 ? 1 : 0; lv < kNumLevels; lv++)
			for (int b = 1; b < 4; b++) {
				const ParsedBand &pb = ps.high[c][lv][b];
				const BandDesc &bd = plan.ch[c].band[lv][b];
				if (!pb.present || pb.width != bd.width || pb.height != bd.height || (pb.offset & 3) || (pb.codebook != 1 && pb.codebook != 0) || (bd.offset & 7) || (bd.pitch & 7)) return false;
				dev::DecBandJob bj = { sample_addr + pb.offset, pb.bytes, coeff_base + bd.offset, bd.height * bd.pitch, pb.quant };
				bands->push_back(bj);
			}
	}
	return true;
}

inline void dec_build_plan(const FramePlan &plan, int out_pixel_kind, dev::DecPlan *dp)
{
	memset(dp, 0, sizeof(*dp));
	dp->width = plan.width; dp->display_height = plan.display_height; dp->encoded_format = plan.encoded_format; dp->num_channels = plan.num_channels;
	struct Key { int area, c, lv, b; };
	std::vector<Key> keys;
	for (int c = 0; c < plan.num_channels; c++) {
		const BandDesc &ll = plan.ch[c].band[2][0];
		dp->low[c] = dev::DecPlanBand{ ll.width, ll.height, ll.pitch, (int)ll.offset };
		dp->low_bias[c] = lowpass_bias(plan.precision, ll.width, out_pixel_kind, c);
		for (int lv = 0; lv < kNumLevels; lv++)
			for (int b = 1; b < 4; b++) {
				const BandDesc &bd = plan.ch[c].band[lv][b];
				dp->high[c][lv][b] = dev::DecPlanBand{ bd.width, bd.height, bd.pitch, (int)bd.offset };
				keys.push_back(Key{ bd.width * bd.height, c, lv, b });
			}
	}
	std::stable_sort(keys.begin(), keys.end(), [](const Key &a, const Key &b) { return a.area > b.area; });
	for (size_t k = 0; k < keys.size(); k++) dp->slot[keys[k].c][keys[k].lv][keys[k].b] = (int)k;
	dp->bands_per_frame = (int)keys.size();
}

inline bool dx_build_jobs(const ParsedSample &ps, const FramePlan &plan, const dev::DecPlan &dp, const uint8_t *sample_addr, int16_t *coeff_base, int out_pixel_kind,
                          int f, int nframes, dev::DecBandJob *table, dev::DecLowpassJob *lowpass , bool skip_level1 = false,
                          dev::DecDiffJob *diff = nullptr )
{
	for (int c = 0; c < plan.num_channels; c++) {
		if (diff) diff[c] = dev::DecDiffJob{ nullptr, 0, 0, 0, nullptr, 0u, 0 };
		const ParsedBand &lp = ps.lowpass[c];
		const BandDesc &ll = plan.ch[c].band[2][0];
		if (!lp.present || lp.width != ll.width || lp.height != ll.height) return false;
		lowpass[c] = dev::DecLowpassJob{ sample_addr + lp.offset, coeff_base + ll.offset, ll.width, ll.height, ll.pitch, lowpass_bias(plan.precision, ll.width, out_pixel_kind, c) };
		for (int lv = 0; lv < kNumLevels; lv++)
			for (int b = 1; b < 4; b++) {
				const ParsedBand &pb = ps.high[c][lv][b];
				const BandDesc &bd = plan.ch[c].band[lv][b];
				dev::DecBandJob &bj = table[(size_t)dp.slot[c][lv][b] * nframes + f];
				bj = dev::DecBandJob{ sample_addr, 0u, coeff_base + bd.offset, bd.height * bd.pitch, 1, 0u, 0 };
				if (skip_level1 && lv == 0) continue;
				if (!pb.present || pb.width != bd.width || pb.height != bd.height || (pb.offset & 3) || pb.codebook < 0 || pb.codebook > 2 || (bd.offset & 7) || (bd.pitch & 7)) return false;
				if ((pb.codebook == 2 || pb.difference) && !diff) return false;
				bj.bits = sample_addr + pb.offset; bj.bytes = pb.bytes; bj.quant = pb.quant; bj.table = pb.codebook == 2;
				if (pb.difference) {
					if (pb.peak_level && (size_t)pb.peak_offset + 2 > ps.size) return false;
					diff[c] = dev::DecDiffJob{ coeff_base + bd.offset, bd.width, bd.height, bd.pitch, pb.peak_level ? sample_addr + pb.peak_offset : nullptr,
					                           pb.peak_level ? (uint32_t)(ps.size - pb.peak_offset) : 0u, pb.peak_level };
				}
			}
	}
	return true;
}

inline dev::DxTilePlan dx_tile_plan(const FramePlan &plan, const dev::DecPlan &dp, int nframes, bool skip_level1 = false, bool level1_block_lists = false, bool interlaced = false, uint32_t tile_max = dev::DX_TILE)
{
	int mask_base[kMaxChannels][kNumBands];
	dec_block_list_layout(plan, mask_base);
	dev::DxTilePlan tp;
	memset(&tp, 0, sizeof(tp));
	tp.nslots = dp.bands_per_frame; tp.nframes = nframes;
	int pos = 0;
	uint32_t cum = 0;
	for (int group = 0; group < 2; group++) {
		for (int c = 0; c < plan.num_channels; c++)
			for (int lv = 0; lv < kNumLevels; lv++) {
				if ((lv == 0) != (group == 1)) continue;
				for (int b = 1; b < 4; b++) {
					const BandDesc &bd = plan.ch[c].band[lv][b];
					const uint32_t n = (uint32_t)(bd.height * bd.pitch);
					const uint32_t per = (skip_level1 && lv == 0) ? 0u : (n + tile_max - 1) / tile_max;
					tp.tile_len[pos] = per ? ((n + per - 1) / per + 511u) / 512u * 512u : tile_max;
					tp.slot_of[pos] = (uint8_t)dp.slot[c][lv][b];
					tp.mask_base[pos] = (level1_block_lists && lv == 0 && !(interlaced && b == 2)) ? mask_base[c][b] : -1;
					tp.cum[pos] = cum; cum += per * (uint32_t)nframes;
					tp.per_band[pos] = per ? per : 1;
					pos++;
				}
			}
		if (group == 0) tp.split = cum;
	}
	tp.total = cum; tp.first = 0;
	return tp;
}

inline uint32_t dx_number_chunks(dev::DecBandJob *jobs, int njobs, std::vector<dev::DxChunkDesc> *chunk_desc)
{
	uint32_t at = 0;
	chunk_desc->clear();
	for (int j = 0; j < njobs; j++) {
		const uint32_t n = (jobs[j].bytes + dev::DX_CHUNK_BYTES - 1) / dev::DX_CHUNK_BYTES;
		jobs[j].chunk0 = at;
		for (uint32_t c = 0; c < n; c++) chunk_desc->push_back(dev::DxChunkDesc{ jobs[j].bits, jobs[j].bytes, c, jobs[j].table, 0u });
		at += n;
	}
	return at;
}

}
```

cineform-sdk_amd/csrc/cfhd_entropy_kernels.h:

```cpp
#pragma once
#include <stdint.h>
#include <cfhd_gfx950.h>

#ifdef CFHD_AMD_PROBES
#define CFHD_PROBE(p) (p)
#else
#define CFHD_PROBE(p) 0
#endif

namespace cfhd {
namespace dev {

#ifndef CFHD_ENT_FILL
#define CFHD_ENT_FILL 16384
#endif
#ifndef CFHD_ENT_PER_THREAD
#define CFHD_ENT_PER_THREAD 16
#endif
#ifndef CFHD_ENT_TOK_CAP
#define CFHD_ENT_TOK_CAP 256
#endif
enum { FWD_CHUNK_COLS_ENT = 496 };
enum { ENT_THREADS = 256, ENT_LANES = 64, ENT_WAVES = ENT_THREADS / ENT_LANES, ENT_PER_THREAD = CFHD_ENT_PER_THREAD, ENT_SEG = ENT_LANES * ENT_PER_THREAD,
       ENT_LDS_WORDS = 256, ENT_TOK_CAP = CFHD_ENT_TOK_CAP, ENT_MAX_HOLES = 60 ,
       ENT_FILL = CFHD_ENT_FILL ,
       ENT_TOK_STRIDE = ENT_SEG, ENT_STR_BITS = 26, ENT_CODE_COMPLEX = 63 ,
       ENT_RUN_COMPLEX = 0xff  };

struct EntTables {
	uint32_t value_code[2048];
	uint32_t run_bits[3072];
	uint16_t run_total[3072];
	uint16_t run_count[3072];
	uint8_t run_size[3072];
	uint32_t band_end_bits; int band_end_size;
	uint2 run_pack[3072];
};

struct EntBandJob {
	const int16_t *coeffs;
	int n;
	int seg_base, nseg;
	int frame, hole;
	int table;
};

struct EntSegJob {
	const int16_t *coeffs;
	int n;
	int first;
	int band;
	int table;
	int pitch;
	int mask_base;
};

struct EntSegState {
	int first_nz, last_nz;
	uint32_t bits;
	int prev_nz;
	uint32_t bitoff;
	uint32_t ntok;
	uint32_t run_code, run_size;
	uint32_t run_bits;
	uint32_t lead32, lead_valid;
	uint8_t *out;
	uint32_t info;
	uint32_t peaks;
};
static_assert(sizeof(EntSegState) == 64, "one segment state per 64 bytes");

struct EntBandState { uint32_t seg_bits, tail_run, payload_bytes, base_byte; uint8_t *out;
                      uint32_t npeaks, pad; uint8_t *peak_out;  };

struct EntHole { int tmpl_offset, kind, fixed_bytes, band_job; const int16_t *lowpass; int lp_width, lp_height, lp_pitch; };
struct EntPatch { int kind, at_tmpl, at_holes, start_tmpl, start_holes, end_tmpl, end_holes, tag; };

struct EntFrameJob {
	uint8_t *out; uint32_t out_cap;
	const uint8_t *tmpl; int tmpl_bytes;
	const uint8_t *word_holes;
	const EntHole *holes; int nholes;
	const EntPatch *patches; int npatches;
	uint32_t *sample_bytes;
	uint32_t *peak_flag;
};

__device__ __forceinline__ uint32_t bswap32(uint32_t v) { return (v >> 24) | ((v >> 8) & 0xff00u) | ((v << 8) & 0xff0000u) | (v << 24); }

__device__ __forceinline__ int block_excl_sum(int v, int *buf, int *total)
{
	const int lane = wave_lane(), wave = (int)(threadIdx.x >> 6);
	const int incl = (int)wave_incl_scan((uint32_t)v);
	if (lane == ENT_LANES - 1) buf[wave] = incl;
	__syncthreads();
	int base = 0, tot = 0;
#pragma unroll
	for (int w = 0; w < ENT_WAVES; w++) { const int x = buf[w]; if (w < wave) base += x; tot += x; }
	if (total) *total = tot;
	__syncthreads();
	return base + incl - v;
}
__device__ __forceinline__ int block_excl_max(int v, int *buf, int *total)
{
	const int lane = wave_lane(), wave = (int)(threadIdx.x >> 6);
	int incl = v;
#pragma unroll
	for (int d = 1; d < ENT_LANES; d <<= 1) { const int x = __shfl_up(incl, (unsigned)d); if (lane >= d && x > incl) incl = x; }
	if (lane == ENT_LANES - 1) buf[wave] = incl;
	int excl = __shfl_up(incl, 1u);
	if (lane == 0) excl = -1;
	__syncthreads();
	int base = -1, tot = -1;
#pragma unroll
	for (int w = 0; w < ENT_WAVES; w++) { const int x = buf[w]; if (w < wave && x > base) base = x; if (x > tot) tot = x; }
	if (total) *total = tot;
	__syncthreads();
	return excl > base ? excl : base;
}

__device__ __forceinline__ uint32_t run_bits_any(const EntTables *T, uint32_t run)
{
	uint32_t bits = 0;
	if (run >= 3072u) {
		const uint32_t c = T->run_count[3071], n = (run - 3072u) / c + 1u;
		bits = n * T->run_size[3071]; run -= n * c;
	}
	return bits + T->run_total[run];
}

__device__ __forceinline__ uint32_t value_entry(const EntTables *T, int v)
{
	v = v < -1023 ? -1023 : (v > 1023 ? 1023 : v);
	return T->value_code[v & 2047];
}

struct EntBatchGeom { int segs_per_frame, bands_per_frame; size_t coeff_stride; };
__device__ __forceinline__ EntSegJob ent_seg_job(const EntSegJob *seg_jobs, const EntBatchGeom &g, int seg, int *frame = nullptr)
{
	const int f = seg / g.segs_per_frame, s = seg - f * g.segs_per_frame;
	if (frame) *frame = f;
	EntSegJob job = seg_jobs[s];
	job.coeffs += (size_t)f * g.coeff_stride; job.band += f * g.bands_per_frame;
	return job;
}

enum { ENT_PEAK_THRESHOLD = 250, ENT_PEAK_OFF_BITS = 21, ENT_PEAK_MAX = (1 << ENT_PEAK_OFF_BITS) - 1,
       ENT_PEAK_TABLE_MAX = 2 * 0xffff };
static_assert(ENT_PEAK_TABLE_MAX <= ENT_PEAK_MAX, "every table that is written has positions for all its peaks");
static_assert(ENT_SEG < (1 << (32 - ENT_PEAK_OFF_BITS)), "a segment's peak count and its position in the band's table share a word");
__device__ __forceinline__ void ent_load_segment(const EntSegJob &job, int lane, uint32_t *w)
{
	const int rem = job.n - job.first;
	const uint32_t *src = (const uint32_t *)(job.coeffs + job.first);
	if (rem >= ENT_SEG) {
#pragma unroll
		for (int j = 0; j < ENT_SEG / 128; j++) w[j] = CFHD_LDG32(src + j * ENT_LANES + lane);
	} else {
#pragma unroll
		for (int j = 0; j < ENT_SEG / 128; j++) {
			const int d = j * ENT_LANES + lane;
			uint32_t x = 2 * d < rem ? CFHD_LDG32(src + d) : 0u;
			if (2 * d + 1 >= rem) x &= 0xffffu;
			w[j] = x;
		}
	}
}

__device__ __forceinline__ void ent_count_tokens(int seg, const EntSegJob &job, int frame, int ntok, int lane, uint32_t *s_tok, EntSegState *segs, const EntTables *tables,
                                                 uint32_t *peak_flags, uint32_t *tokens, int probe);

__device__ __forceinline__ void ent_count_segment(int seg, const EntSegJob &job, int frame, const uint32_t *w, int lane, uint32_t *s_tok, EntSegState *segs, const EntTables *tables,
                                                  uint32_t *peak_flags, uint32_t *tokens, int probe)
{
	if (CFHD_PROBE(probe) == 1) { uint32_t o = 0; for (int j = 0; j < ENT_SEG / 128; j++) o |= w[j]; const unsigned long long q = __ballot(o == 0x12345u); if (lane == 0) { EntSegState &z = segs[seg]; z.first_nz = -1; z.last_nz = -1; z.bits = q == 0x123456789ull; z.ntok = 0; z.lead32 = 0; z.lead_valid = 0; } return; }
	int ntok = 0;
#pragma unroll
	for (int j = 0; j < ENT_SEG / 128; j++) {
		const uint32_t vl = w[j] & 0xffffu, vh = w[j] >> 16;
		const unsigned long long ml = __ballot(vl != 0u), mh = __ballot(vh != 0u);
		const int pl = ntok + (int)wave_mbcnt(ml) + (int)wave_mbcnt(mh);
		const uint32_t idx = (uint32_t)(j * 128 + 2 * lane) << 16;
		if (vl) s_tok[pl] = idx | vl;
		if (vh) s_tok[pl + (vl != 0u)] = (idx + 0x10000u) | vh;
		ntok += __popcll(ml) + __popcll(mh);
	}
	CFHD_WAVE_SYNC();
	ent_count_tokens(seg, job, frame, ntok, lane, s_tok, segs, tables, peak_flags, tokens, probe);
}

__device__ __forceinline__ void ent_count_tokens(int seg, const EntSegJob &job, int frame, int ntok, int lane, uint32_t *s_tok, EntSegState *segs, const EntTables *tables,
                                                 uint32_t *peak_flags, uint32_t *tokens, int probe)
{
	const EntTables *T = tables + job.table;
	uint32_t bits = 0, lead32 = 0, lead_valid = 0;
	if (CFHD_PROBE(probe) == 2) { const unsigned long long q = __ballot(s_tok[lane] == 0x12345u); if (lane == 0) { EntSegState &z = segs[seg]; z.first_nz = -1; z.last_nz = -1; z.bits = q == 0x123456789ull && ntok == 0x12345; z.ntok = 0; z.lead32 = 0; z.lead_valid = 0; } return; }
	uint32_t npeaks = 0;
	for (int t0 = 0; t0 < ntok; t0 += ENT_LANES) {
		const int t = t0 + lane;
		const bool have = t < ntok;
		const uint32_t tok = have ? s_tok[t] : 0u;
		const uint32_t before = (have && t > 0) ? s_tok[t - 1] : 0u;
		const uint32_t run = (have && t > 0) ? (tok >> 16) - (before >> 16) - 1u : 0u;
		int value = (int)(int16_t)(tok & 0xffffu);
		const bool is_peak = job.table && (value > ENT_PEAK_THRESHOLD || value < -ENT_PEAK_THRESHOLD);
		if (is_peak) value = value > 0 ? ENT_PEAK_THRESHOLD + 1 : -ENT_PEAK_THRESHOLD - 1;
		npeaks += (uint32_t)__popcll(__ballot(is_peak));
		const uint32_t ve = value_entry(T, value);
		const uint32_t rt = T->run_total[run];
		const uint2 rp = T->run_pack[run];
		uint32_t my_top = 0, my_len = 0;
		if (have) {
			bits += rt + (ve >> 27);
			uint32_t *seg_out = tokens + (size_t)seg * ENT_TOK_STRIDE;
			const uint32_t vs = ve >> 27, vc = ve & 0x7FFFFFFu, rs = run ? rp.y & 0xffu : 0u;
			const bool simple = (run == 0u || (rp.y >> 8) == run) && rs + vs <= (uint32_t)ENT_STR_BITS;
			const uint32_t str = simple ? (((run ? rp.x : 0u) << vs) | vc) << (32u - rs - vs) : 0u;
			const uint32_t len = simple ? rs + vs : (uint32_t)ENT_CODE_COMPLEX;
			const uint32_t rec = simple ? str | len : (run << 22) | (((uint32_t)value & 0xffffu) << 6) | len;
			if (CFHD_PROBE(probe) != 4) seg_out[t] = rec;
			my_top = str; my_len = len;
		}
		if (t0 == 0) {
			const int hi = ntok < ENT_LANES ? ntok : ENT_LANES;
			const unsigned long long cx = __ballot(have && my_len == (uint32_t)ENT_CODE_COMPLEX);
			const uint32_t l = (have && my_len != (uint32_t)ENT_CODE_COMPLEX) ? my_len : 0u;
			const uint32_t sc = wave_incl_scan(l), ex = sc - l;
			const int stop_lane = cx ? __builtin_ctzll(cx) : hi;
			uint32_t part = (lane < stop_lane && ex < 32u) ? my_top >> ex : 0u;
#pragma unroll
			for (int d = 1; d < ENT_LANES; d <<= 1) part |= __shfl_xor(part, d);
			lead32 = part;
			const uint32_t known = stop_lane > 0 ? wave_get(sc, stop_lane - 1) : 0u;
			lead_valid = known < 32u ? known : 32u;
		}
	}
	if (npeaks && lane == 0) atomic_or_u32(&peak_flags[frame], 1u);
	bits = wave_get(wave_incl_scan(bits), ENT_LANES - 1);
	if (lane == 0) {
		EntSegState &s = segs[seg];
		s.first_nz = ntok ? job.first + (int)(s_tok[0] >> 16) : -1;
		s.last_nz = ntok ? job.first + (int)(s_tok[ntok - 1] >> 16) : -1;
		s.bits = bits;
		s.ntok = (uint32_t)ntok;
		s.lead32 = lead32; s.lead_valid = lead_valid;
		s.out = nullptr;
		s.info = (job.first != 0 ? 1u : 0u) | (job.first + ENT_SEG < job.n ? 2u : 0u) | ((uint32_t)job.table << 8);
		s.peaks = npeaks;
	}
}

enum { ENT_COUNT_SEGS = 1 };
__global__ void __launch_bounds__(ENT_THREADS) k_ent_count(const EntSegJob *seg_jobs, EntBatchGeom geom, int total_segs, EntSegState *segs, const EntTables *tables,
                                                            uint32_t *peak_flags, uint32_t *tokens, int range_lo, int range_n,
                                                            int probe = 0 )
{
	__shared__ uint32_t s_tok_all[ENT_WAVES][ENT_SEG];
	const int lane = wave_lane();
	const int wave = wave_uniform((int)(threadIdx.x >> 6));
	const int idx0 = wave_uniform(((int)blockIdx.x * ENT_WAVES + wave) * ENT_COUNT_SEGS);
	if (idx0 >= total_segs) return;
	const int seg0 = (idx0 / range_n) * geom.segs_per_frame + range_lo + idx0 % range_n;
	static_assert(ENT_COUNT_SEGS == 1, "the range mapping takes one segment per wave");
	EntSegJob job[ENT_COUNT_SEGS]; int frame[ENT_COUNT_SEGS];
	uint32_t w[ENT_COUNT_SEGS][ENT_SEG / 128];
#pragma unroll
	for (int k = 0; k < ENT_COUNT_SEGS; k++)
		if (idx0 + k < total_segs) { job[k] = ent_seg_job(seg_jobs, geom, seg0 + k, &frame[k]); ent_load_segment(job[k], lane, w[k]); }
#pragma unroll
	for (int k = 0; k < ENT_COUNT_SEGS; k++)
		if (idx0 + k < total_segs) {
			ent_count_segment(seg0 + k, job[k], frame[k], w[k], lane, s_tok_all[wave], segs, tables, peak_flags, tokens, probe);
			CFHD_WAVE_SYNC();
		}
}

struct EntBlockLists { const uint4 *blocks; const unsigned long long *masks; const int16_t *coeff0; size_t masks_per_frame; };
__global__ void __launch_bounds__(ENT_THREADS) k_ent_count_blocks(const EntSegJob *seg_jobs, EntBatchGeom geom, int total_segs, EntSegState *segs, const EntTables *tables,
                                                                   uint32_t *peak_flags, uint32_t *tokens, int range_lo, int range_n, EntBlockLists lists)
{
	__shared__ uint32_t s_tok_all[ENT_WAVES][ENT_SEG];
	const int lane = wave_lane();
	const int wave = wave_uniform((int)(threadIdx.x >> 6));
	const int idx0 = wave_uniform((int)blockIdx.x * ENT_WAVES + wave);
	if (idx0 >= total_segs) return;
	const int seg = (idx0 / range_n) * geom.segs_per_frame + range_lo + idx0 % range_n;
	int frame;
	const EntSegJob job = ent_seg_job(seg_jobs, geom, seg, &frame);
	uint32_t *s_tok = s_tok_all[wave];
	const int pitch = job.pitch, cpr = (pitch + FWD_CHUNK_COLS_ENT - 1) / FWD_CHUNK_COLS_ENT;
	const int end = job.first + ENT_SEG < job.n ? job.first + ENT_SEG : job.n;
	const uint4 *blocks = wave_uniform_ptr(lists.blocks + (size_t)(job.coeffs - lists.coeff0) / 8);
	const unsigned long long *masks = wave_uniform_ptr(lists.masks + (size_t)frame * lists.masks_per_frame + job.mask_base);
	const int row0 = job.first / pitch, col0 = job.first - row0 * pitch;
	uint32_t entry[2]; bool listed[2];
#pragma unroll
	for (int h = 0; h < 2; h++) {
		const int q = lane + 64 * h, pos = job.first + 8 * q;
		int row = row0, col = col0 + 8 * q;
		while (col >= pitch) { col -= pitch; row++; }
		static_assert(FWD_CHUNK_COLS_ENT == 62 * 8, "the division below is by 62 blocks");
		const uint32_t c8 = (uint32_t)col >> 3, k = mul_u24(c8, 1058u) >> 16, i = c8 - mul_u24(k, 62u);
		unsigned long long m = 0ull;
		if (pos < end) m = masks[mul_u24((uint32_t)row, (uint32_t)cpr) + k];
		listed[h] = ((m >> i) & 1ull) != 0ull;
		entry[h] = ((mul_u24((uint32_t)row, (uint32_t)pitch >> 3) + mul_u24(k, 62u) + (uint32_t)__popcll(m & ((1ull << i) - 1ull))) << 7) | (uint32_t)q;
	}
	const unsigned long long b0 = __ballot(listed[0]), b1 = __ballot(listed[1]);
	const int n0 = __popcll(b0), nlisted = n0 + __popcll(b1);
	if (listed[0]) s_tok[wave_mbcnt(b0)] = entry[0];
	if (listed[1]) s_tok[n0 + (int)wave_mbcnt(b1)] = entry[1];
	CFHD_WAVE_SYNC();
	const uint32_t mine[2] = { lane < nlisted ? s_tok[lane] : 0u, lane + 64 < nlisted ? s_tok[lane + 64] : 0u };
	CFHD_WAVE_SYNC();
	int ntok = 0;
#pragma unroll
	for (int h = 0; h < 2; h++) {
		if (64 * h >= nlisted) break;
		uint32_t w[4] = { 0u, 0u, 0u, 0u };
		if (lane + 64 * h < nlisted) { const cfhd_u4 v = CFHD_LDG128(&blocks[mine[h] >> 7]); w[0] = v.x; w[1] = v.y; w[2] = v.z; w[3] = v.w; }
		uint32_t cnt = 0;
#pragma unroll
		for (int d = 0; d < 4; d++) cnt += ((w[d] & 0xffffu) != 0u) + ((w[d] >> 16) != 0u);
		const uint32_t incl = wave_incl_scan(cnt);
		uint32_t p = (uint32_t)ntok + incl - cnt;
		const uint32_t local = 8u * (mine[h] & 127u);
#pragma unroll
		for (int d = 0; d < 4; d++) {
			const uint32_t vl = w[d] & 0xffffu, vh = w[d] >> 16;
			if (vl) s_tok[p++] = ((local + 2u * d) << 16) | vl;
			if (vh) s_tok[p++] = ((local + 2u * d + 1u) << 16) | vh;
		}
		ntok += (int)wave_get(incl, ENT_LANES - 1);
	}
	CFHD_WAVE_SYNC();
	ent_count_tokens(seg, job, frame, ntok, lane, s_tok, segs, tables, peak_flags, tokens, 0);
}

__global__ void __launch_bounds__(ENT_THREADS) k_ent_scan(const EntBandJob *bands, EntSegState *segs, EntBandState *band_state, const EntTables *tables)
{
	enum { ENT_SCAN_PER = 4 };
	__shared__ int s_scan[ENT_THREADS];
	const EntBandJob &job = bands[blockIdx.x];
	const EntTables *T = tables + job.table;
	int carry_prev = -1; uint32_t carry_bits = 0, carry_peaks = 0;
	for (int c0 = 0; c0 < job.nseg; c0 += ENT_THREADS * ENT_SCAN_PER) {
		const int i0 = c0 + (int)threadIdx.x * ENT_SCAN_PER;
		EntSegState s[ENT_SCAN_PER];
#pragma unroll
		for (int k = 0; k < ENT_SCAN_PER; k++) {
			s[k].first_nz = -1; s[k].last_nz = -1; s[k].bits = 0; s[k].lead32 = 0; s[k].lead_valid = 0; s[k].peaks = 0;
			if (i0 + k < job.nseg) s[k] = segs[job.seg_base + i0 + k];
		}
		int mine = -1;
#pragma unroll
		for (int k = 0; k < ENT_SCAN_PER; k++) mine = s[k].last_nz > mine ? s[k].last_nz : mine;
		int chunk_last;
		int prev = block_excl_max(mine, s_scan, &chunk_last);
		if (prev < carry_prev) prev = carry_prev;
		int prevs[ENT_SCAN_PER]; uint32_t bits[ENT_SCAN_PER], rcode[ENT_SCAN_PER], rsize[ENT_SCAN_PER], rbits[ENT_SCAN_PER];
#pragma unroll
		for (int k = 0; k < ENT_SCAN_PER; k++) { prevs[k] = prev; prev = s[k].last_nz > prev ? s[k].last_nz : prev; }
		uint32_t total = 0;
#pragma unroll
		for (int k = 0; k < ENT_SCAN_PER; k++) {
			bits[k] = s[k].bits;
			rcode[k] = 0u; rsize[k] = 0u; rbits[k] = 0u;
			if (s[k].first_nz >= 0) {
				const uint32_t run = (uint32_t)(s[k].first_nz - prevs[k] - 1);
				rbits[k] = run_bits_any(T, run);
				bits[k] += rbits[k];
				if (run > 0u && run < 3072u && T->run_count[run] == run) { rcode[k] = T->run_bits[run]; rsize[k] = T->run_size[run]; }
				else if (run > 0u) rsize[k] = (uint32_t)ENT_RUN_COMPLEX;
				const uint32_t rs = rsize[k];
				if (rs == (uint32_t)ENT_RUN_COMPLEX) { s[k].lead32 = 0u; s[k].lead_valid = 0u; }
				else if (rs) {
					s[k].lead32 = (rcode[k] << (32u - rs)) | (s[k].lead32 >> rs);
					s[k].lead_valid = s[k].lead_valid + rs < 32u ? s[k].lead_valid + rs : 32u;
				}
			}
			total += bits[k];
		}
		int chunk_bits;
		uint32_t off = carry_bits + (uint32_t)block_excl_sum((int)total, s_scan, &chunk_bits);
		uint32_t pk_off = 0; int chunk_peaks = 0;
		if (job.table) {
			uint32_t mine_pk = 0;
#pragma unroll
			for (int k = 0; k < ENT_SCAN_PER; k++) mine_pk += s[k].peaks;
			pk_off = carry_peaks + (uint32_t)block_excl_sum((int)mine_pk, s_scan, &chunk_peaks);
		}
#pragma unroll
		for (int k = 0; k < ENT_SCAN_PER; k++) {
			if (i0 + k < job.nseg) {
				EntSegState &o = segs[job.seg_base + i0 + k];
				o.prev_nz = prevs[k]; o.bits = bits[k]; o.bitoff = off; o.run_code = rcode[k]; o.run_size = rsize[k]; o.run_bits = rbits[k]; o.lead32 = s[k].lead32; o.lead_valid = s[k].lead_valid;
				if (job.table) o.peaks = (s[k].peaks << ENT_PEAK_OFF_BITS) | (pk_off < (uint32_t)ENT_PEAK_MAX ? pk_off : (uint32_t)ENT_PEAK_MAX);
			}
			off += bits[k]; pk_off += s[k].peaks;
		}
		carry_peaks += (uint32_t)chunk_peaks;
		if (chunk_last > carry_prev) carry_prev = chunk_last;
		carry_bits += (uint32_t)chunk_bits;
	}
	if (threadIdx.x == 0) {
		EntBandState &b = band_state[blockIdx.x];
		b.seg_bits = carry_bits;
		b.tail_run = (uint32_t)(job.n - 1 - carry_prev);
		uint32_t bits = carry_bits + run_bits_any(T, b.tail_run) + (uint32_t)T->band_end_size;
		b.payload_bytes = ((bits + 31u) >> 5) << 2;
		b.base_byte = 0; b.out = nullptr;
		b.npeaks = carry_peaks; b.pad = 0; b.peak_out = nullptr;
	}
}

__device__ __forceinline__ void put_code_plain(uint32_t *words, uint64_t pos, uint32_t code, int size)
{
	if (!size) return;
	const uint64_t v = (uint64_t)code << (64 - size - (int)(pos & 31));
	uint32_t *w = words + (pos >> 5);
	w[0] |= bswap32((uint32_t)(v >> 32));
	const uint32_t lo = (uint32_t)v;
	if (lo) w[1] |= bswap32(lo);
}

__global__ void __launch_bounds__(ENT_THREADS) k_ent_layout(const EntFrameJob *frames, const EntBandJob *bands, EntSegState *segs,
                                                             EntBandState *band_state, const EntTables *tables)
{
	const EntFrameJob &f = frames[blockIdx.x];
	const int part = blockIdx.y, nparts = gridDim.y;
	__shared__ uint32_t s_cum[ENT_MAX_HOLES + 1];
	__shared__ uint32_t s_piece[ENT_MAX_HOLES + 1];
	__shared__ int s_ok;
	const int tid = threadIdx.x;
	if (tid < 64) {
		uint32_t bytes = 0;
		if (tid < f.nholes) {
			const EntHole &hole = f.holes[tid];
			if (hole.kind == 0) bytes = (uint32_t)hole.fixed_bytes;
			else if (hole.kind == 1) bytes = band_state[hole.band_job].payload_bytes;
			else {
				const uint32_t np = band_state[hole.band_job].npeaks;
				bytes = (np && np <= (uint32_t)ENT_PEAK_TABLE_MAX) ? 4u + 4u * ((np + 1u) >> 1) : 0u;
			}
		}
		const uint32_t pieces = tid < f.nholes ? (bytes / ENT_FILL ? bytes / ENT_FILL : 1u) : 0u;
		const uint32_t cum = wave_incl_scan(bytes), pc = wave_incl_scan(pieces);
		if (tid <= f.nholes && tid <= ENT_MAX_HOLES) { s_cum[tid] = cum - bytes; s_piece[tid] = pc - pieces; }
		const uint32_t total = (uint32_t)f.tmpl_bytes + wave_get(cum, 63);
		if (tid == 0) { s_ok = total <= f.out_cap; if (part == 0) *f.sample_bytes = total <= f.out_cap ? total : 0u; }
	}
	__syncthreads();
	if (!s_ok) return;
	uint32_t *out = (uint32_t *)f.out;
	const uint32_t *tw = (const uint32_t *)f.tmpl;
	if (part == 0) for (int i = tid; i < f.tmpl_bytes / 4; i += ENT_THREADS) out[i + (s_cum[f.word_holes[i]] >> 2)] = tw[i];
	__syncthreads();
	for (int i = tid; part == 0 && i < f.npatches; i += ENT_THREADS) {
		const EntPatch &p = f.patches[i];
		const uint32_t at = (uint32_t)p.at_tmpl + s_cum[p.at_holes], end = (uint32_t)p.end_tmpl + s_cum[p.end_holes];
		if (p.kind == 0) {
			uint32_t size = (end - at) >> 2; size = size ? size - 1 : 0;
			int tag = p.tag;
			if (tag & 0x2000) { tag |= (int)((size >> 16) & 0xff); size &= 0xffff; } else size &= 0xffff;
			tag = -tag;
			out[at >> 2] = bswap32(((uint32_t)(uint16_t)tag << 16) | size);
		} else if (p.kind == 2) {
			if (s_cum[p.start_holes + 1] != s_cum[p.start_holes]) {
				const uint32_t offset = end - at;
				out[at >> 2] = bswap32(((uint32_t)(uint16_t)(-75) << 16) | (offset & 0xffffu));
				out[(at >> 2) + 1] = bswap32(((uint32_t)(uint16_t)(-76) << 16) | (offset >> 16));
				out[(at >> 2) + 2] = bswap32(((uint32_t)(uint16_t)(-74) << 16) | ((uint32_t)(ENT_PEAK_THRESHOLD * p.tag) & 0xffffu));
			}
		} else {
			const uint32_t start = (uint32_t)p.start_tmpl + s_cum[p.start_holes];
			out[at >> 2] = bswap32(end - start);
		}
	}
	const uint32_t npieces = s_piece[f.nholes];
	int h = 0;
	for (uint32_t p = (uint32_t)part; p < npieces; p += (uint32_t)nparts) {
		while (s_piece[h + 1] <= p) h++;
		const EntHole &hole = f.holes[h];
		const uint32_t base = (uint32_t)hole.tmpl_offset + s_cum[h], bytes = s_cum[h + 1] - s_cum[h];
		const uint32_t k = p - s_piece[h], last = s_piece[h + 1] - s_piece[h] - 1;
		const uint32_t w0 = k * (ENT_FILL / 4), w1 = k == last ? bytes / 4 : w0 + ENT_FILL / 4;
		if (hole.kind == 0) {
			const int count = hole.lp_width * hole.lp_height;
			for (uint32_t i = w0 + tid; i < w1; i += ENT_THREADS) {
				uint32_t w = 0;
#pragma unroll
				for (int q = 0; q < 2; q++) {
					const int e = 2 * (int)i + q;
					uint32_t v = 0;
					if (e < count) { const int r = e / hole.lp_width, c = e - r * hole.lp_width; v = (uint16_t)hole.lowpass[(size_t)r * hole.lp_pitch + c]; }
					w = (w << 16) | v;
				}
				out[(base >> 2) + i] = bswap32(w);
			}
			continue;
		}
		if (hole.kind == 2) {
			const uint32_t np = band_state[hole.band_job].npeaks;
			for (uint32_t i = w0 + tid; i < w1; i += ENT_THREADS) out[(base >> 2) + i] = i == 0 ? bswap32(((uint32_t)(uint16_t)(-0x4001) << 16) | ((np + 1u) >> 1)) : 0u;
			if (k == 0 && tid == 0) band_state[hole.band_job].peak_out = bytes ? f.out + base + 4 : nullptr;
			continue;
		}
		const EntBandState bs = band_state[hole.band_job];
		const uint32_t tail_word = (uint32_t)(bs.seg_bits >> 5) < bytes / 4 ? (uint32_t)(bs.seg_bits >> 5) : bytes / 4;
		for (uint32_t i = w0 + tid; i < (w1 < tail_word ? w1 : tail_word); i += ENT_THREADS) out[(base >> 2) + i] = 0;
		if (k != last) continue;
		const EntTables *T = tables + bands[hole.band_job].table;
		const uint32_t maxc = T->run_count[3071], maxs = T->run_size[3071], maxb = T->run_bits[3071];
		const uint32_t copies = bs.tail_run >= 3071u ? (bs.tail_run - 3071u) / maxc + 1u : 0u;
		const uint64_t p0 = bs.seg_bits, p1 = p0 + (uint64_t)copies * maxs;
		uint32_t *words = out + (base >> 2);
		for (uint32_t i = tail_word + tid; i < bytes / 4; i += ENT_THREADS) {
			uint32_t w = 0;
			const uint64_t lo = (uint64_t)i * 32u, hi = lo + 32u;
			if (copies && hi > p0 && lo < p1) {
				uint64_t j = lo > p0 ? (lo - p0) / maxs : 0u;
				for (; j < copies && p0 + j * maxs < hi; j++) {
					const int64_t sh = (int64_t)(hi - (p0 + j * maxs)) - (int64_t)maxs;
					w |= sh >= 0 ? (sh < 32 ? maxb << sh : 0u) : maxb >> (-sh);
				}
			}
			words[i] = bswap32(w);
		}
		__syncthreads();
		for (int i = tid; i < bands[hole.band_job].nseg; i += ENT_THREADS) segs[bands[hole.band_job].seg_base + i].out = f.out + base;
		if (tid == 0) {
			EntBandState &b = band_state[hole.band_job];
			b.base_byte = base; b.out = f.out + base;
			uint64_t pos = p1;
			uint32_t run = bs.tail_run - copies * maxc;
			while (run > 0) {
				const uint32_t idx = run < 3072 ? run : 3071;
				put_code_plain(words, pos, T->run_bits[idx], T->run_size[idx]);
				pos += T->run_size[idx];
				run -= T->run_count[idx];
			}
			put_code_plain(words, pos, T->band_end_bits, T->band_end_size);
		}
	}
}

__device__ __forceinline__ void ent_put_string(uint32_t *s_words, uint32_t *out, bool use_lds, uint32_t first_word, uint64_t pos, uint64_t str)
{
	const uint32_t sh = (uint32_t)pos & 31u, w = (uint32_t)(pos >> 5);
	const uint64_t top = str >> sh;
	const uint32_t a = (uint32_t)(top >> 32), b = (uint32_t)top, c = (uint32_t)(((uint64_t)(uint32_t)str << 32) >> sh);
	if (use_lds) {
		atomic_or_u32(&s_words[w - first_word], a);
		if (b) atomic_or_u32(&s_words[w - first_word + 1], b);
		if (c) atomic_or_u32(&s_words[w - first_word + 2], c);
	} else {
		atomic_or_u32(&out[w], bswap32(a));
		if (b) atomic_or_u32(&out[w + 1], bswap32(b));
		if (c) atomic_or_u32(&out[w + 2], bswap32(c));
	}
}

__device__ __forceinline__ void ent_put_string32(uint32_t *s_words, uint32_t *out, bool use_lds, uint32_t first_word, uint64_t pos, uint32_t str)
{
	const uint32_t sh = (uint32_t)pos & 31u, w = (uint32_t)(pos >> 5);
	const uint32_t a = str >> sh, b = sh ? str << (32u - sh) : 0u;
	if (use_lds) {
		atomic_or_u32(&s_words[w - first_word], a);
		if (b) atomic_or_u32(&s_words[w - first_word + 1], b);
	} else {
		atomic_or_u32(&out[w], bswap32(a));
		if (b) atomic_or_u32(&out[w + 1], bswap32(b));
	}
}

__device__ __forceinline__ void ent_put_long_run(const EntTables *T, uint32_t *s_words, uint32_t *out, bool use_lds, uint32_t first_word, uint64_t pos, uint32_t run, int owner)
{
	const int lane = wave_lane();
	const uint32_t cmax = T->run_count[3071], smax = T->run_size[3071], codemax = T->run_bits[3071];
	const uint32_t nrep = run >= 3072u ? (run - 3072u) / cmax + 1u : 0u;
	for (uint32_t i = (uint32_t)lane; i < nrep; i += ENT_LANES) ent_put_string(s_words, out, use_lds, first_word, pos + (uint64_t)i * smax, (uint64_t)codemax << (64u - smax));
	if (lane == owner) {
		uint32_t left = run - nrep * cmax;
		pos += (uint64_t)nrep * smax;
		while (left > 0u) {
			const uint2 rc = T->run_pack[left < 3072u ? left : 3071u];
			const uint32_t size = rc.y & 0xffu;
			ent_put_string(s_words, out, use_lds, first_word, pos, (uint64_t)rc.x << (64u - size));
			pos += size; left -= rc.y >> 8;
		}
	}
}

__device__ __forceinline__ bool ent_ordinary(const EntSegState &st)
{
	return st.bits >= 32u && (uint32_t)((st.bitoff + st.bits - 1u) >> 5) - (uint32_t)(st.bitoff >> 5) + 1u <= (uint32_t)ENT_LDS_WORDS;
}
__device__ __forceinline__ bool ent_neighbours_merge(const EntSegState &a, const EntSegState &b)
{
	const uint32_t o = b.bitoff & 31u;
	return o != 0u && ent_ordinary(a) && ent_ordinary(b) && b.lead_valid >= 32u - o;
}

__device__ __forceinline__ void ent_emit_segment(const EntSegState &st, const EntSegState &pv, const EntSegState &nx, const uint32_t first_rec, const uint32_t *seg_str, int lane,
                                                 uint32_t *s_words, const EntTables *tables, int probe)
{
	if (st.bits == 0) return;
	const EntTables *T = tables + (st.info >> 8);
	const bool has_prev = (st.info & 1u) != 0u, has_next = (st.info & 2u) != 0u;
	const bool prev_writes_first = has_prev && ent_neighbours_merge(pv, st);
	const bool merge_next = has_next && ent_neighbours_merge(st, nx);
	uint32_t *out = (uint32_t *)st.out;
	if (!out) return;
	if (CFHD_PROBE(probe) == 2) { if (first_rec == 0x12345u && lane == 0) out[0] = 1; return; }
	const int ntok = (int)st.ntok;
	const uint64_t seg_pos = st.bitoff;
	const uint32_t first_word = (uint32_t)(seg_pos >> 5), last_word = (uint32_t)((seg_pos + st.bits - 1) >> 5);
	const uint32_t nwords = last_word - first_word + 1;
	const bool use_lds = nwords <= ENT_LDS_WORDS;
	if (use_lds) for (int i = lane; i < (int)nwords + 2; i += ENT_LANES) s_words[i] = 0;
	CFHD_WAVE_SYNC();
	if (st.run_size == (uint32_t)ENT_RUN_COMPLEX) ent_put_long_run(T, s_words, out, use_lds, first_word, seg_pos, (uint32_t)(st.first_nz - st.prev_nz - 1), 0);
	else if (st.run_size && lane == 0) ent_put_string(s_words, out, use_lds, first_word, seg_pos, (uint64_t)st.run_code << (64u - st.run_size));
	uint64_t round_pos = seg_pos + st.run_bits;
	for (int t = lane, t0 = 0; t0 < ntok; t0 += ENT_LANES, t += ENT_LANES) {
		const bool have = t < ntok;
		uint32_t rec = t0 == 0 ? first_rec : seg_str[have ? t : 0];
		if (!have) rec = 0u;
		uint32_t len = rec & 63u;
		const bool complex = len == (uint32_t)ENT_CODE_COMPLEX;
		uint32_t run = 0, ve = 0;
		if (__ballot(complex)) {
			if (complex) {
				run = rec >> 22;
				ve = value_entry(T, (int)(int16_t)((rec >> 6) & 0xffffu));
				len = (uint32_t)T->run_total[run] + (ve >> 27);
			}
		}
		const uint32_t sc = wave_incl_scan(len);
		uint64_t pos = round_pos + (sc - len);
		round_pos += wave_get(sc, ENT_LANES - 1);
		if (have && !complex) ent_put_string32(s_words, out, use_lds, first_word, pos, rec & ~63u);
		if (complex) {
			uint32_t left = run;
			while (left > 0u) {
				const uint2 rc = T->run_pack[left];
				const uint32_t size = rc.y & 0xffu;
				ent_put_string(s_words, out, use_lds, first_word, pos, (uint64_t)rc.x << (64u - size));
				pos += size; left -= rc.y >> 8;
			}
			ent_put_string(s_words, out, use_lds, first_word, pos, (uint64_t)(ve & 0x7FFFFFFu) << (64u - (ve >> 27)));
		}
	}
	CFHD_WAVE_SYNC();
	if (CFHD_PROBE(probe) == 3) { if (s_words[lane] == 0x12345u) out[0] = 1; return; }
	if (use_lds) {
		const bool first_shared = (seg_pos & 31u) != 0u, last_shared = ((seg_pos + st.bits) & 31u) != 0u;
		for (int i = lane; i < (int)nwords; i += ENT_LANES) {
			uint32_t w = s_words[i];
			const bool is_first = i == 0, is_last = i == (int)nwords - 1;
			if (is_first && prev_writes_first) continue;
			if (is_last && merge_next) w |= nx.lead32 >> ((seg_pos + st.bits) & 31u);
			w = bswap32(w);
			if (((is_first && first_shared) || (is_last && last_shared && !merge_next)) && CFHD_PROBE(probe) != 4) { if (w) atomic_or_u32(&out[first_word + i], w); }
			else if (CFHD_PROBE(probe) != 5) out[first_word + i] = w;
		}
	}
}

enum { ENT_EMIT_SEGS = 1 };
__global__ void __launch_bounds__(ENT_THREADS) k_ent_emit(int total_segs, const EntSegState *segs, const EntTables *tables, const uint32_t *tokens,
                                                           int probe = 0 )
{
	__shared__ uint32_t s_words_all[ENT_WAVES][ENT_LDS_WORDS + 3];
	if (CFHD_PROBE(probe) == 1) return;
	const int lane = wave_lane();
	const int wave = wave_uniform((int)(threadIdx.x >> 6));
	const int seg0 = wave_uniform(((int)blockIdx.x * ENT_WAVES + wave) * ENT_EMIT_SEGS);
	if (seg0 >= total_segs) return;
	uint32_t first_rec[ENT_EMIT_SEGS];
	EntSegState st[ENT_EMIT_SEGS + 2];
#pragma unroll
	for (int k = 0; k < ENT_EMIT_SEGS; k++) {
		const int sg = seg0 + k < total_segs ? seg0 + k : seg0;
		first_rec[k] = tokens[(size_t)sg * ENT_TOK_STRIDE + lane];
	}
#pragma unroll
	for (int k = 0; k < ENT_EMIT_SEGS + 2; k++) {
		int sg = seg0 - 1 + k;
		sg = sg < 0 ? 0 : (sg < total_segs ? sg : total_segs - 1);
		st[k] = segs[sg];
	}
#pragma unroll
	for (int k = 0; k < ENT_EMIT_SEGS; k++)
		if (seg0 + k < total_segs) {
			ent_emit_segment(st[k + 1], st[k], st[k + 2], first_rec[k], tokens + (size_t)(seg0 + k) * ENT_TOK_STRIDE, lane, s_words_all[wave], tables, probe);
			CFHD_WAVE_SYNC();
		}
}


struct EntPeakHoles { int n; int hole[7]; };
__global__ void __launch_bounds__(ENT_THREADS) k_ent_peaks(const EntFrameJob *frames, EntPeakHoles which, const EntBandJob *bands, const EntSegJob *seg_jobs, EntBatchGeom geom,
                                                            const EntSegState *segs, const EntBandState *band_state)
{
	const EntHole &hole = frames[blockIdx.z].holes[which.hole[blockIdx.y]];
	const int bj = hole.band_job, quant = hole.fixed_bytes;
	const EntBandState bs = band_state[bj];
	if (!bs.npeaks || !bs.peak_out || bs.npeaks > (uint32_t)ENT_PEAK_TABLE_MAX) return;
	const EntBandJob band = bands[bj];
	int16_t *table = (int16_t *)bs.peak_out;
	const int lane = wave_lane();
	const int wave = wave_uniform((int)(threadIdx.x >> 6));
	for (int sg = (int)blockIdx.x * ENT_WAVES + wave; sg < band.nseg; sg += (int)gridDim.x * ENT_WAVES) {
		const uint32_t pk = segs[band.seg_base + sg].peaks;
		if (!(pk >> ENT_PEAK_OFF_BITS)) continue;
		int frame;
		const EntSegJob job = ent_seg_job(seg_jobs, geom, band.seg_base + sg, &frame);
		uint32_t w[ENT_SEG / 128];
		ent_load_segment(job, lane, w);
		uint32_t at = pk & (uint32_t)ENT_PEAK_MAX;
#pragma unroll
		for (int j = 0; j < ENT_SEG / 128; j++) {
			const int vl = (int)(int16_t)(w[j] & 0xffffu), vh = (int)(int16_t)(w[j] >> 16);
			const bool pl = vl > ENT_PEAK_THRESHOLD || vl < -ENT_PEAK_THRESHOLD, ph = vh > ENT_PEAK_THRESHOLD || vh < -ENT_PEAK_THRESHOLD;
			const unsigned long long ml = __ballot(pl), mh = __ballot(ph);
			const uint32_t mine = at + wave_mbcnt(ml) + wave_mbcnt(mh);
			if (pl) table[mine] = (int16_t)(vl * quant);
			if (ph) table[mine + (pl ? 1u : 0u)] = (int16_t)(vh * quant);
			at += (uint32_t)(__popcll(ml) + __popcll(mh));
		}
	}
}

__global__ void __launch_bounds__(ENT_THREADS) k_ent_pack_offsets(const uint32_t *sizes, int n, uint32_t *offsets)
{
	__shared__ int s_scan[ENT_THREADS];
	uint32_t carry = 0;
	for (int c0 = 0; c0 < n; c0 += ENT_THREADS) {
		const int i = c0 + (int)threadIdx.x;
		const uint32_t sz = i < n ? (sizes[i] + 63u) & ~63u : 0u;
		int total;
		const uint32_t off = carry + (uint32_t)block_excl_sum((int)sz, s_scan, &total);
		if (i < n) offsets[i] = off;
		carry += (uint32_t)total;
	}
	if (threadIdx.x == 0) offsets[n] = carry;
}

__global__ void __launch_bounds__(ENT_THREADS) k_ent_pack(const uint8_t *samples, size_t stride, const uint32_t *sizes, const uint32_t *offsets, uint8_t *packed)
{
	const int f = blockIdx.y;
	const uint4 *src = (const uint4 *)(samples + stride * (size_t)f);
	uint4 *dst = (uint4 *)(packed + offsets[f]);
	const uint32_t n16 = (sizes[f] + 15u) >> 4;
	for (uint32_t i = blockIdx.x * ENT_THREADS + threadIdx.x; i < n16; i += gridDim.x * ENT_THREADS) dst[i] = src[i];
}

enum { DEC_K1 = 12, DEC_THREADS = 64 };

struct DecMulti {
	uint16_t pre_bits;
	int16_t v1;
	uint16_t mid_post;
	int16_t v2;
};

struct DecTables {
	DecMulti multi[1 << DEC_K1];
	uint32_t lut1[1 << DEC_K1];
	uint32_t lut2_size;
	uint32_t lut2[1];
};

struct DecBandJob {
	const uint8_t *bits; uint32_t bytes;
	int16_t *dst; int n;
	int quant;
	uint32_t chunk0;
	int table;
};

struct DecDiffJob { int16_t *band; int width, height, pitch; const uint8_t *peaks; uint32_t peak_bytes; int level; };

struct DecLowpassJob { const uint8_t *src; int16_t *dst; int width, height, pitch, bias; };

__global__ void __launch_bounds__(DEC_THREADS) k_dec_bands(const DecBandJob *jobs, int njobs, const DecTables *T, int *errors)
{
	__shared__ uint2 s_multi[1 << DEC_K1];
	for (int i = threadIdx.x; i < (1 << DEC_K1); i += DEC_THREADS) s_multi[i] = ((const uint2 *)T->multi)[i];
	__syncthreads();
	const int j = blockIdx.x * DEC_THREADS + threadIdx.x;
	if (j >= njobs) return;
	const DecBandJob job = jobs[j];
	const uint32_t *words = (const uint32_t *)job.bits;
	const uint32_t nwords = job.bytes >> 2;
	uint32_t w0 = nwords > 0 ? words[0] : 0u, w1 = nwords > 1 ? words[1] : 0u, w2 = nwords > 2 ? words[2] : 0u, w3 = nwords > 3 ? words[3] : 0u;
	uint32_t wpos = 0;
	uint64_t acc = 0; int have = 0;
	int idx = 0, err = 0;
	const int quant = job.quant, n = job.n;
	for (;;) {
		if (have <= 32) {
			const uint32_t w = bswap32(w0);
			w0 = w1; w1 = w2; w2 = w3;
			w3 = (wpos + 4 < nwords) ? words[wpos + 4] : 0u;
			wpos++;
			acc |= (uint64_t)w << (32 - have);
			have += 32;
		}
		const uint2 m = s_multi[(uint32_t)(acc >> (64 - DEC_K1))];
		const int used = (int)(m.x & 15u);
		if (used) {
			const int pre = (int)((m.x >> 4) & 0xfffu), v1 = (int)(int16_t)(m.x >> 16);
			const int mid = (int)(m.y & 0xffu), post = (int)((m.y >> 8) & 0xffu), v2 = (int)(int16_t)(m.y >> 16);
			acc <<= used; have -= used;
			idx += pre;
			if (v1) { if (idx >= n) { err = 2; break; } job.dst[idx++] = (int16_t)(v1 * quant); }
			idx += mid;
			if (v2) { if (idx >= n) { err = 2; break; } job.dst[idx++] = (int16_t)(v2 * quant); }
			idx += post;
			if (idx > n) { err = 2; break; }
		} else {
			uint32_t e = T->lut1[(uint32_t)(acc >> (64 - DEC_K1))];
			if ((e & 31u) == 31u) {
				const int nb = (int)((e >> 5) & 31u);
				e = T->lut2[(e >> 10) + (uint32_t)((acc << DEC_K1) >> (64 - nb))];
			}
			const int len = (int)(e & 31u);
			if (len == 0) { err = 1; break; }
			acc <<= len; have -= len;
			const uint32_t mag = e >> 16;
			if (mag == 0xffffu) break;
			if (mag) {
				const int negative = (int)(acc >> 63);
				acc <<= 1; have -= 1;
				if (idx >= n) { err = 2; break; }
				const int v = (int)mag * quant;
				job.dst[idx++] = (int16_t)(negative ? -v : v);
			} else { idx += (int)((e >> 5) & 0x7ffu); if (idx > n) { err = 2; break; } }
		}
		if (wpos > nwords + 6) { err = 3; break; }
	}
	if (err) atomic_or_u32((uint32_t *)errors, 1u);
}

enum { DECP_THREADS = 256, DECP_SUB_BITS = 256, DECP_LL_THREADS = 512, DECP_LL_SUB_BITS = 128 };
enum : uint32_t { DECP_END = 0xFFFFFFFFu, DECP_BAD = 0xFFFFFFFEu };

template <int NT>
__device__ __forceinline__ uint32_t decp_excl_sum(uint32_t v, uint32_t *s_wsum , uint32_t *total)
{
	const int t = threadIdx.x, wave = t >> 6, lane = t & 63;
	const uint32_t incl = wave_incl_scan(v);
	__syncthreads();
	if (lane == 63) s_wsum[wave] = incl;
	__syncthreads();
	uint32_t before = 0, all = 0;
#pragma unroll
	for (int w = 0; w < NT / 64; w++) { const uint32_t x = s_wsum[w]; if (w < wave) before += x; all += x; }
	*total = all;
	return before + incl - v;
}

struct DecSub { uint32_t end, cnt; };

template <bool WRITE>
__device__ __forceinline__ DecSub dec_sub(const uint32_t *s_words, const uint32_t *s_lut1, const DecTables *T, uint32_t p, const uint32_t limit,
                                          int16_t *dst, uint32_t idx, const uint32_t n, const int quant)
{
	uint32_t wi = p >> 5;
	const int sh = (int)(p & 31u);
	uint64_t acc = (((uint64_t)s_words[wi] << 32) | s_words[wi + 1]) << sh;
	int have = 64 - sh;
	wi += 2;
	uint32_t cnt = 0;
	while (p < limit) {
		if (have < 32) { acc |= (uint64_t)s_words[wi++] << (32 - have); have += 32; }
		uint32_t e = s_lut1[(uint32_t)(acc >> (64 - DEC_K1))];
		if ((e & 31u) == 31u) {
			const int nb = (int)((e >> 5) & 31u);
			e = T->lut2[(e >> 10) + (uint32_t)((acc << DEC_K1) >> (64 - nb))];
		}
		int len = (int)(e & 31u);
		if (len == 0) return DecSub{ DECP_BAD, cnt };
		const uint32_t mag = e >> 16;
		if (mag == 0xffffu) return DecSub{ DECP_END, cnt };
		if (mag) {
			if (WRITE) {
				const int negative = (int)((acc << len) >> 63);
				const int v = (int)mag * quant;
				if (idx + cnt < n) dst[idx + cnt] = (int16_t)(negative ? -v : v);
			}
			len++; cnt++;
		} else cnt += (e >> 5) & 0x7ffu;
		acc <<= len; have -= len; p += (uint32_t)len;
	}
	return DecSub{ p, cnt };
}

template <int NT, int SUB_BITS>
__device__ __forceinline__ void dec_bands_par(const DecBandJob *jobs, const DecTables *T, int *errors)
{
	enum { DECP_THREADS = NT, DECP_SUB_BITS = SUB_BITS, DECP_SEQ_BITS = NT * SUB_BITS, DECP_SEQ_WORDS = DECP_SEQ_BITS / 32 };
	__shared__ uint32_t s_lut1[1 << DEC_K1];
	__shared__ uint32_t s_words[DECP_SEQ_WORDS + 4];
	__shared__ uint32_t s_end[DECP_THREADS];
	__shared__ uint32_t s_wsum[DECP_THREADS / 64];
	__shared__ int s_flag[2];
	const int t = threadIdx.x;
	const DecBandJob job = jobs[blockIdx.x];
	const uint32_t *words = (const uint32_t *)job.bits;
	const uint32_t nwords = job.bytes >> 2, n = (uint32_t)job.n;
	for (int i = t; i < (1 << DEC_K1); i += DECP_THREADS) s_lut1[i] = T->lut1[i];
	if (t < 2) s_flag[t] = 0;
	{
		uint4 *z = (uint4 *)job.dst;
		const uint4 zero = { 0u, 0u, 0u, 0u };
		for (uint32_t i = t; i < n / 8; i += DECP_THREADS) z[i] = zero;
	}
	uint32_t carry = 0, base_idx = 0;
	int err = 0;
	for (uint32_t seq0 = 0; ; seq0 += DECP_SEQ_WORDS) {
		if (seq0 >= nwords) { err = 3; break; }
		__syncthreads();
		for (int i = t; i < DECP_SEQ_WORDS + 4; i += DECP_THREADS) { const uint32_t w = seq0 + (uint32_t)i; s_words[i] = w < nwords ? bswap32(words[w]) : 0u; }
		__syncthreads();
		const uint64_t left = (uint64_t)(nwords - seq0) * 32u;
		const uint32_t seq_bits = left < (uint64_t)DECP_SEQ_BITS ? (uint32_t)left : (uint32_t)DECP_SEQ_BITS;
		const int nsub = (int)((seq_bits + DECP_SUB_BITS - 1) / DECP_SUB_BITS);
		const bool active = t < nsub;
		uint32_t start = t ? (uint32_t)t * DECP_SUB_BITS : carry;
		const uint32_t limit = (uint32_t)(t + 1) * DECP_SUB_BITS < seq_bits ? (uint32_t)(t + 1) * DECP_SUB_BITS : seq_bits;
		DecSub r = active ? dec_sub<false>(s_words, s_lut1, T, start, limit, nullptr, 0u, 0u, 0) : DecSub{ DECP_END, 0u };
		for (int round = 0; ; round++) {
			s_end[t] = r.end;
			__syncthreads();
			if (t == 0) s_flag[(round + 1) & 1] = 0;
			const uint32_t ns = t ? s_end[t - 1] : start;
			const bool changed = active && ns != start;
			if (changed) s_flag[round & 1] = 1;
			__syncthreads();
			if (!s_flag[round & 1]) break;
			if (changed) {
				start = ns;
				if (ns >= DECP_BAD) { r.end = ns; r.cnt = 0; }
				else r = dec_sub<false>(s_words, s_lut1, T, start, limit, nullptr, 0u, 0u, 0);
			}
		}
		uint32_t total;
		const uint32_t my_idx = base_idx + decp_excl_sum<NT>(r.cnt, s_wsum, &total);
		const uint32_t last = s_end[nsub - 1];
		if (last == DECP_BAD) { err = 1; break; }
		if (total > n - base_idx) { err = 2; break; }
		if (active && start < DECP_BAD && r.cnt) (void)dec_sub<true>(s_words, s_lut1, T, start, r.end, job.dst, my_idx, n, job.quant);
		if (last == DECP_END) break;
		if (seq_bits < (uint32_t)DECP_SEQ_BITS) { err = 3; break; }
		carry = last - DECP_SEQ_BITS;
		base_idx += total;
	}
	if (err && t == 0) atomic_or_u32((uint32_t *)errors, 1u << err);
}
__global__ void __launch_bounds__(DECP_THREADS) k_dec_bands_par(const DecBandJob *jobs, const DecTables *T, int *errors) { dec_bands_par<DECP_THREADS, DECP_SUB_BITS>(jobs, T, errors); }
__global__ void __launch_bounds__(DECP_LL_THREADS) k_dec_bands_par_ll(const DecBandJob *jobs, const DecTables *T, int *errors) { dec_bands_par<DECP_LL_THREADS, DECP_LL_SUB_BITS>(jobs, T, errors); }

struct DecPlanBand { int width, height, pitch, offset; };
struct DecPlan {
	int width, display_height, encoded_format, num_channels, bands_per_frame;
	DecPlanBand low[4]; int low_bias[4];
	DecPlanBand high[4][3][4];
	int slot[4][3][4];
};
enum { DEC_PARSE_THREADS = 64, DEC_ERR_PARSE = 0x100 };

struct DecTagReader {
	const uint8_t *d; uint64_t base; uint32_t w; int lane;
	__device__ __forceinline__ uint32_t word(uint64_t pos)
	{
		const uint64_t b = pos & ~(uint64_t)255;
		if (b != base) { w = *(const uint32_t *)(d + b + 4 * (size_t)lane); base = b; }
		return bswap32(wave_read(w, (int)((pos >> 2) & 63u)));
	}
};

__global__ void __launch_bounds__(DEC_PARSE_THREADS) k_dec_parse(const uint8_t *samples, size_t sample_stride, const uint32_t *sizes, int nframes, const DecPlan *P,
                                                                 int16_t *coeffs, size_t coeff_stride, DecBandJob *bandjobs, DecLowpassJob *lowjobs, int *errors,
                                                                 DecDiffJob *diffjobs )
{
	const int f = blockIdx.x;
	const int lane = wave_lane();
	const bool writer = lane == 0;
	const uint8_t *d = samples + sample_stride * (size_t)f;
	int16_t *cbase = coeffs + coeff_stride * (size_t)f;
	const uint64_t size = sizes[f];
	const int nch = P->num_channels;
	if (writer) for (int c = 0; c < nch; c++) {
		lowjobs[f * nch + c] = DecLowpassJob{ d, cbase + P->low[c].offset, 0, 0, P->low[c].pitch, 0 };
		for (int lv = 0; lv < 3; lv++)
			for (int b = 1; b < 4; b++) {
				const DecPlanBand pb = P->high[c][lv][b];
				bandjobs[(size_t)P->slot[c][lv][b] * nframes + f] = DecBandJob{ d, 0u, cbase + pb.offset, pb.height * pb.pitch, 1 };
			}
	}
	DecTagReader rd; rd.d = d; rd.base = ~(uint64_t)0; rd.w = 0; rd.lane = lane;
	uint64_t pos = 0, pending_at = 0, peak_base = 0;
	uint32_t pending = 0, seen_low = 0, peak_offset = 0;
	int peak_level = 0;
	if (writer && diffjobs) for (int c = 0; c < nch; c++) diffjobs[f * nch + c] = DecDiffJob{ nullptr, 0, 0, 0, nullptr, 0u, 0 };
	uint64_t seen = 0;
	int channel = 0, lv = -1, band = 0, bw = 0, bh = 0, bq = 1, bflags = 0, lw = 0, lh = 0;
	int width = 0, height = 0, display_height = 0, num_channels = 0, encoded_format = 0;
	bool bad = size < 4;
	while (!bad && pos + 4 <= size) {
		const uint32_t word = rd.word(pos);
		int tag = (int)(int16_t)(word >> 16);
		const int value = (int)(word & 0xffffu);
		if (tag < 0) tag = -tag;
		pos += 4;
		if (tag & 0x4000) {
			const uint32_t bytes = (tag & 0x2000) ? ((((uint32_t)(tag & 0xff) << 16) | (uint32_t)value) * 4u) : (uint32_t)value * 4u;
			if (pos + bytes > size) { bad = true; break; }
			pos += bytes;
			continue;
		}
		if (tag & 0x2000) {
			if ((tag & 0xff00) == 0x2000) { pending = ((((uint32_t)(tag & 0xff)) << 16) | (uint32_t)value) * 4u; pending_at = pos; }
			continue;
		}
		switch (tag) {
		case 2: pos += 4u * (uint64_t)value; break;
		case 62: channel = value; if (channel >= 4) bad = true; break;
		case 12: num_channels = value; break;
		case 84: encoded_format = value; break;
		case 20: width = value; break;
		case 21: height = value; break;
		case 85: display_height = value; break;
		case 27: lw = value; break;
		case 28: lh = value; break;
		case 4:
			if (value == 0x0f0f) {
				const uint64_t end = pending_at + pending;
				const uint64_t bytes = (uint64_t)lw * (uint64_t)lh * 2u;
				if (pending == 0 || pos + bytes > end || end > size || channel >= nch) { bad = true; break; }
				const DecPlanBand ll = P->low[channel];
				if (lw != ll.width || lh != ll.height) { bad = true; break; }
				if (writer) lowjobs[f * nch + channel] = DecLowpassJob{ d + pos, cbase + ll.offset, ll.width, ll.height, ll.pitch, P->low_bias[channel] };
				seen_low |= 1u << channel;
				pos = end; pending = 0;
			}
			break;
		case 38: lv = value - 1; if (lv < 0 || lv >= 3) bad = true; break;
		case 48: band = value; if (band < 1 || band > 3) bad = true; bflags = 0; break;
		case 72: bflags = value; break;
		case 75: peak_offset = (peak_offset & ~0xffffu) | (uint32_t)value; peak_base = pos; peak_level = 0; break;
		case 76: peak_offset = (peak_offset & 0xffffu) | ((uint32_t)value << 16); peak_level = 0; break;
		case 74: peak_level = value; break;
		case 49: bw = value; break;
		case 50: bh = value; break;
		case 53: bq = value; break;
		case 55: {
			const uint64_t end = pending_at + pending;
			if (lv < 0 || pending == 0 || end < pos + 4 || end > size || channel >= nch || band < 1) { bad = true; break; }
			const DecPlanBand pb = P->high[channel][lv][band];
			const int codebook = bflags & 0xf;
			const bool difference = (bflags >> 4) & 1;
			if (bw != pb.width || bh != pb.height || (pos & 3u) || codebook > 2 || ((codebook == 2 || difference) && !diffjobs)) { bad = true; break; }
			if (peak_level && peak_base + peak_offset + 2 > size) { bad = true; break; }
			if (writer) bandjobs[(size_t)P->slot[channel][lv][band] * nframes + f] = DecBandJob{ d + pos, (uint32_t)(end - 4 - pos), cbase + pb.offset, pb.height * pb.pitch, bq, 0u, codebook == 2 };
			if (writer && difference) diffjobs[f * nch + channel] = DecDiffJob{ cbase + pb.offset, pb.width, pb.height, pb.pitch, peak_level ? d + peak_base + peak_offset : nullptr,
			                                                                    peak_level ? (uint32_t)(size - (peak_base + peak_offset)) : 0u, peak_level };
			peak_level = 0;
			seen |= (uint64_t)1 << ((channel * 3 + lv) * 3 + band - 1);
			pos = end; pending = 0;
			break; }
		default: break;
		}
	}
	if (display_height == 0) display_height = height;
	const uint64_t want = ((uint64_t)1 << (nch * 9)) - 1u;
	if (bad || width != P->width || display_height != P->display_height || encoded_format != P->encoded_format || num_channels != nch
	    || seen != want || seen_low != (1u << nch) - 1u) {
		if (writer) for (int c = 0; c < nch; c++)
			for (int l = 0; l < 3; l++)
				for (int b = 1; b < 4; b++) bandjobs[(size_t)P->slot[c][l][b] * nframes + f].bytes = 0u;
		if (writer) atomic_or_u32((uint32_t *)errors, (uint32_t)DEC_ERR_PARSE);
	}
}

__global__ void __launch_bounds__(256) k_dec_lowpass(const DecLowpassJob *jobs)
{
	const DecLowpassJob job = jobs[blockIdx.y];
	const int count = job.width * job.height;
	for (int i = blockIdx.x * 256 + threadIdx.x; i < count; i += gridDim.x * 256) {
		const int r = i / job.width, c = i - r * job.width;
		int v = (int)(int16_t)(((uint32_t)job.src[2 * i] << 8) | job.src[2 * i + 1]);
		if (job.width & 1) v = (int)(uint16_t)v;
		v += job.bias;
		job.dst[(size_t)r * job.pitch + c] = (int16_t)(v > 0x7fff ? 0x7fff : v);
	}
}

}
}
```

Baseline: 63240.

## Use longer variable-length entropy segments for level-1 block-list bands

Level-1 luma bands that use block lists now get longer segments (default 4096 coefficients, overridable through an environment variable). Each segment walks several block spans and counts tokens in windows, carrying run state across them. Token storage becomes variable-sized per segment with per-frame offsets, and the token record format changes to allow longer runs. The emit LDS buffer grows to fit the larger segments. The aim is fewer segments, less per-segment scan and emit overhead, and fewer shared boundary words, at the cost of less parallelism and more LDS per wave.

Result: faster. 66530, median of 6 (+5.2%).

```diff
diff --git a/cineform-sdk_amd/csrc/cfhd_entropy_gpu.h b/cineform-sdk_amd/csrc/cfhd_entropy_gpu.h
--- a/cineform-sdk_amd/csrc/cfhd_entropy_gpu.h
+++ b/cineform-sdk_amd/csrc/cfhd_entropy_gpu.h
@@ -55,7 +55,7 @@
 	bool group_ = false; GopPlan gplan_;
 	FramePlan plan_; int n_ = 0, active_ = 0, device_ = 0 ; size_t cap_ = 0; void *stream_ = nullptr;
 	int active_frames() const { return active_ > 0 && active_ < n_ ? active_ : n_; }
-	int nbands_ = 0, total_segs_ = 0;
+	int nbands_ = 0, total_segs_ = 0; size_t tok_per_frame_ = 0;
 	std::vector<SampleTemplate> tmpl_;
 	uint8_t *d_samples_ = nullptr, *h_samples_ = nullptr;
 	uint32_t *d_sizes_ = nullptr, *h_sizes_ = nullptr;
diff --git a/cineform-sdk_amd/csrc/cfhd_entropy_gpu.hip b/cineform-sdk_amd/csrc/cfhd_entropy_gpu.hip
--- a/cineform-sdk_amd/csrc/cfhd_entropy_gpu.hip
+++ b/cineform-sdk_amd/csrc/cfhd_entropy_gpu.hip
@@ -75,17 +75,20 @@
 	build_template(hdr0, &tmpl_[0]);
 	EntHostJobs &jobs = host_->jobs;
 	host_->geom = group_ ? ent_hole_geometry(gplan_, tmpl_[0]) : ent_hole_geometry(plan, tmpl_[0]);
-	if (!ent_build_band_jobs(host_->geom, tmpl_[0], n_, d_coeffs, stride, &jobs)) return -3;
-	nbands_ = jobs.nbands; total_segs_ = (int)jobs.segjobs.size();
+	const bool lists = !group_ && !plan.interlaced && plan.encoded_format == ENC_YUV422 && (plan.pixel_kind == PIX_YUY2 || plan.pixel_kind == PIX_2VUY) && plan.width % 32 == 0;
+	static const int l1_seg_env = [] { const char *e = getenv("CFHD_AMD_L1_SEG"); const int v = e ? atoi(e) : 0;
+	                                   return v >= dev::ENT_SEG && v <= dev::ENT_SEG_MAX && v % dev::ENT_SEG == 0 ? v : (int)dev::ENT_SEG_L1; }();
+	if (!ent_build_band_jobs(host_->geom, tmpl_[0], n_, d_coeffs, stride, &jobs, lists ? l1_seg_env : (int)dev::ENT_SEG)) return -3;
+	nbands_ = jobs.nbands; total_segs_ = (int)jobs.segjobs.size(); tok_per_frame_ = jobs.tok_per_frame;
 	HIPCHK(hipMalloc(&d_bands_, jobs.bands.size() * sizeof(dev::EntBandJob)));
 	HIPCHK(hipMemcpy(d_bands_, jobs.bands.data(), jobs.bands.size() * sizeof(dev::EntBandJob), hipMemcpyHostToDevice));
 	HIPCHK(hipMalloc(&d_segband_, jobs.segjobs.size() * sizeof(dev::EntSegJob)));
 	HIPCHK(hipMemcpy(d_segband_, jobs.segjobs.data(), jobs.segjobs.size() * sizeof(dev::EntSegJob), hipMemcpyHostToDevice));
 	HIPCHK(hipMalloc(&d_segs_, jobs.segjobs.size() * sizeof(dev::EntSegState)));
-	HIPCHK(hipMalloc(&d_tokens_, jobs.segjobs.size() * (size_t)dev::ENT_TOK_STRIDE * sizeof(uint32_t)));
+	HIPCHK(hipMalloc(&d_tokens_, jobs.tok_per_frame * (size_t)n_ * sizeof(uint32_t)));
 	HIPCHK(hipMalloc(&d_bandstate_, jobs.bands.size() * sizeof(dev::EntBandState)));
 	static_assert((int)kBlockChunkCols == (int)dev::FWD_CHUNK_COLS_ENT, "one chunk geometry");
-	if (!group_ && !plan.interlaced && plan.encoded_format == ENC_YUV422 && (plan.pixel_kind == PIX_YUY2 || plan.pixel_kind == PIX_2VUY) && plan.width % 32 == 0) {
+	if (lists) {
 		int mask_base[kMaxChannels][kNumBands];
 		masks_per_frame_ = (size_t)block_list_layout(plan, mask_base);
 		HIPCHK(hipMalloc(&d_blocks_, stride * 2 * (size_t)n_));
@@ -134,7 +137,7 @@
 		dirty_ = false;
 	}
 	const dev::EntTables *T = (const dev::EntTables *)d_tables_;
-	const dev::EntBatchGeom geom = { total_segs_ / n_, nbands_, coeff_stride_ };
+	const dev::EntBatchGeom geom = { total_segs_ / n_, nbands_, coeff_stride_, tok_per_frame_ };
 	const int act = active_frames(), total_segs = total_segs_ / n_ * act;
 	(void)hipGetLastError();
 	HIPCHK(hipEventRecord((hipEvent_t)ev_[0], st));
diff --git a/cineform-sdk_amd/csrc/cfhd_entropy_jobs.h b/cineform-sdk_amd/csrc/cfhd_entropy_jobs.h
--- a/cineform-sdk_amd/csrc/cfhd_entropy_jobs.h
+++ b/cineform-sdk_amd/csrc/cfhd_entropy_jobs.h
@@ -195,12 +195,15 @@
 	return true;
 }
 
+static_assert(((size_t)dev::ENT_BLK_SPAN + 2u * (size_t)kMaxFrameDim) / 8u < ((size_t)1 << 23) && dev::ENT_BLK_SPAN / 8 <= 512, "block slot << 9 | block number fits 32 bits");
+
 struct EntHostJobs {
 	std::vector<dev::EntBandJob> bands;
 	std::vector<dev::EntSegJob> segjobs;
 	std::vector<int> band_of_hole;
 	int nbands = 0;
 	std::vector<std::pair<int, int>> ranges_l1, ranges_rest;
+	size_t tok_per_frame = 0;
 };
 
 struct EntHoleGeom { size_t offset; int width, height, pitch; int table ; int mask_base ; bool level1; };
@@ -227,20 +230,25 @@
 	return g;
 }
 
-inline bool ent_build_band_jobs(const std::vector<EntHoleGeom> &geom, const SampleTemplate &t0, int nframes, int16_t *coeffs, size_t stride, EntHostJobs *out)
+inline bool ent_build_band_jobs(const std::vector<EntHoleGeom> &geom, const SampleTemplate &t0, int nframes, int16_t *coeffs, size_t stride, EntHostJobs *out,
+                                int l1_seg = dev::ENT_SEG)
 {
 	if ((int)t0.holes.size() > dev::ENT_MAX_HOLES || (int)t0.patches.size() > kEntMaxPatches || geom.size() != t0.holes.size()) return false;
+	if (l1_seg < dev::ENT_SEG || l1_seg > dev::ENT_SEG_MAX || l1_seg % dev::ENT_SEG) return false;
 	out->bands.clear(); out->segjobs.clear(); out->ranges_l1.clear(); out->ranges_rest.clear();
+	out->tok_per_frame = 0;
 	out->band_of_hole.assign(t0.holes.size(), -1);
 	for (int f = 0; f < nframes; f++) {
 		int16_t *base = coeffs + (size_t)f * stride;
+		size_t tok_at = 0;
 		for (size_t h = 0; h < t0.holes.size(); h++) {
 			const SampleTemplate::Hole &hole = t0.holes[h];
 			if (hole.kind != 1) continue;
 			const EntHoleGeom &bd = geom[h];
 			dev::EntBandJob j;
 			j.coeffs = base + bd.offset; j.n = bd.height * bd.pitch;
-			j.nseg = (j.n + dev::ENT_SEG - 1) / dev::ENT_SEG; j.seg_base = (int)out->segjobs.size();
+			const int len = bd.level1 && bd.table == 0 && bd.mask_base >= 0 ? l1_seg : (int)dev::ENT_SEG;
+			j.nseg = (j.n + len - 1) / len; j.seg_base = (int)out->segjobs.size();
 			j.frame = f; j.hole = (int)h;
 			j.table = bd.table;
 			if (f == 0) {
@@ -248,16 +256,22 @@
 				std::vector<std::pair<int, int>> &r = bd.level1 ? out->ranges_l1 : out->ranges_rest;
 				if (!r.empty() && r.back().first + r.back().second == j.seg_base) r.back().second += j.nseg; else r.push_back({ j.seg_base, j.nseg });
 			}
-			for (int s = 0; s < j.nseg; s++) out->segjobs.push_back(dev::EntSegJob{ j.coeffs, j.n, s * dev::ENT_SEG, (int)out->bands.size(), j.table, bd.pitch, bd.mask_base });
+			for (int s = 0; s < j.nseg; s++) {
+				const int first = s * len, slots = ((j.n - first < len ? j.n - first : len) + dev::ENT_TOK_STRIDE - 1) / dev::ENT_TOK_STRIDE * dev::ENT_TOK_STRIDE;
+				out->segjobs.push_back(dev::EntSegJob{ j.coeffs, j.n, first, (int)out->bands.size(), j.table, bd.pitch, bd.mask_base, len, (int)tok_at });
+				tok_at += (size_t)slots;
+			}
 			out->bands.push_back(j);
 		}
+		if (tok_at > (size_t)INT32_MAX) return false;
+		out->tok_per_frame = tok_at;
 	}
 	out->nbands = (int)out->bands.size() / nframes;
 	return true;
 }
-inline bool ent_build_band_jobs(const FramePlan &plan, const SampleTemplate &t0, int nframes, int16_t *coeffs, size_t stride, EntHostJobs *out)
-{
-	return ent_build_band_jobs(ent_hole_geometry(plan, t0), t0, nframes, coeffs, stride, out);
+inline bool ent_build_band_jobs(const FramePlan &plan, const SampleTemplate &t0, int nframes, int16_t *coeffs, size_t stride, EntHostJobs *out, int l1_seg = dev::ENT_SEG)
+{
+	return ent_build_band_jobs(ent_hole_geometry(plan, t0), t0, nframes, coeffs, stride, out, l1_seg);
 }
 
 inline bool ent_fill_frame_block(const std::vector<EntHoleGeom> &geom, const SampleTemplate &t, int f, const EntHostJobs &jobs, const int16_t *coeffs_f, uint8_t *block)
diff --git a/cineform-sdk_amd/csrc/cfhd_entropy_kernels.h b/cineform-sdk_amd/csrc/cfhd_entropy_kernels.h
--- a/cineform-sdk_amd/csrc/cfhd_entropy_kernels.h
+++ b/cineform-sdk_amd/csrc/cfhd_entropy_kernels.h
@@ -22,10 +22,14 @@
 #endif
 enum { FWD_CHUNK_COLS_ENT = 496 };
 enum { ENT_THREADS = 256, ENT_LANES = 64, ENT_WAVES = ENT_THREADS / ENT_LANES, ENT_PER_THREAD = CFHD_ENT_PER_THREAD, ENT_SEG = ENT_LANES * ENT_PER_THREAD,
-       ENT_LDS_WORDS = 256, ENT_TOK_CAP = CFHD_ENT_TOK_CAP, ENT_MAX_HOLES = 60 ,
+       ENT_LDS_WORDS = 1024, ENT_TOK_CAP = CFHD_ENT_TOK_CAP, ENT_MAX_HOLES = 60 ,
        ENT_FILL = CFHD_ENT_FILL ,
        ENT_TOK_STRIDE = ENT_SEG, ENT_STR_BITS = 26, ENT_CODE_COMPLEX = 63 ,
-       ENT_RUN_COMPLEX = 0xff  };
+       ENT_RUN_COMPLEX = 0xff ,
+       ENT_SEG_L1 = 4096, ENT_SEG_MAX = 8192, ENT_BLK_SPAN = 4096,
+       ENT_REC_RUN_SHIFT = 17 };
+static_assert(ENT_SEG_MAX - 1 < (1 << (32 - ENT_REC_RUN_SHIFT)), "the longest run inside a segment fits the token record's run field");
+static_assert(ENT_SEG_L1 % ENT_SEG == 0 && ENT_SEG_MAX % ENT_SEG == 0 && ENT_BLK_SPAN % ENT_SEG == 0 && ENT_BLK_SPAN / 8 <= 8 * ENT_LANES, "segments are whole token windows; a span is 8 blocks per lane");
 
 struct EntTables {
 	uint32_t value_code[2048];
@@ -53,6 +57,8 @@
 	int table;
 	int pitch;
 	int mask_base;
+	int len;
+	int tok_base;
 };
 
 struct EntSegState {
@@ -64,6 +70,7 @@
 	uint32_t run_code, run_size;
 	uint32_t run_bits;
 	uint32_t lead32, lead_valid;
+	uint32_t tok_blk;
 	uint8_t *out;
 	uint32_t info;
 	uint32_t peaks;
@@ -135,13 +142,14 @@
 	return T->value_code[v & 2047];
 }
 
-struct EntBatchGeom { int segs_per_frame, bands_per_frame; size_t coeff_stride; };
-__device__ __forceinline__ EntSegJob ent_seg_job(const EntSegJob *seg_jobs, const EntBatchGeom &g, int seg, int *frame = nullptr)
+struct EntBatchGeom { int segs_per_frame, bands_per_frame; size_t coeff_stride; size_t tok_per_frame; };
+__device__ __forceinline__ EntSegJob ent_seg_job(const EntSegJob *seg_jobs, const EntBatchGeom &g, int seg, int *frame = nullptr, size_t *tok_base = nullptr)
 {
 	const int f = seg / g.segs_per_frame, s = seg - f * g.segs_per_frame;
 	if (frame) *frame = f;
 	EntSegJob job = seg_jobs[s];
 	job.coeffs += (size_t)f * g.coeff_stride; job.band += f * g.bands_per_frame;
+	if (tok_base) *tok_base = (size_t)f * (g.tok_per_frame ? g.tok_per_frame : (size_t)g.segs_per_frame * ENT_TOK_STRIDE) + (size_t)job.tok_base;
 	return job;
 }
 
@@ -149,10 +157,11 @@
        ENT_PEAK_TABLE_MAX = 2 * 0xffff };
 static_assert(ENT_PEAK_TABLE_MAX <= ENT_PEAK_MAX, "every table that is written has positions for all its peaks");
 static_assert(ENT_SEG < (1 << (32 - ENT_PEAK_OFF_BITS)), "a segment's peak count and its position in the band's table share a word");
-__device__ __forceinline__ void ent_load_segment(const EntSegJob &job, int lane, uint32_t *w)
-{
-	const int rem = job.n - job.first;
-	const uint32_t *src = (const uint32_t *)(job.coeffs + job.first);
+__device__ __forceinline__ void ent_load_segment(const EntSegJob &job, int lane, uint32_t *w, int off = 0)
+{
+	const int span = job.n - job.first < job.len ? job.n - job.first : job.len;
+	const int rem = span - off;
+	const uint32_t *src = (const uint32_t *)(job.coeffs + job.first + off);
 	if (rem >= ENT_SEG) {
 #pragma unroll
 		for (int j = 0; j < ENT_SEG / 128; j++) w[j] = CFHD_LDG32(src + j * ENT_LANES + lane);
@@ -167,62 +176,42 @@
 	}
 }
 
-__device__ __forceinline__ void ent_count_tokens(int seg, const EntSegJob &job, int frame, int ntok, int lane, uint32_t *s_tok, EntSegState *segs, const EntTables *tables,
-                                                 uint32_t *peak_flags, uint32_t *tokens, int probe);
-
-__device__ __forceinline__ void ent_count_segment(int seg, const EntSegJob &job, int frame, const uint32_t *w, int lane, uint32_t *s_tok, EntSegState *segs, const EntTables *tables,
-                                                  uint32_t *peak_flags, uint32_t *tokens, int probe)
-{
-	if (CFHD_PROBE(probe) == 1) { uint32_t o = 0; for (int j = 0; j < ENT_SEG / 128; j++) o |= w[j]; const unsigned long long q = __ballot(o == 0x12345u); if (lane == 0) { EntSegState &z = segs[seg]; z.first_nz = -1; z.last_nz = -1; z.bits = q == 0x123456789ull; z.ntok = 0; z.lead32 = 0; z.lead_valid = 0; } return; }
-	int ntok = 0;
-#pragma unroll
-	for (int j = 0; j < ENT_SEG / 128; j++) {
-		const uint32_t vl = w[j] & 0xffffu, vh = w[j] >> 16;
-		const unsigned long long ml = __ballot(vl != 0u), mh = __ballot(vh != 0u);
-		const int pl = ntok + (int)wave_mbcnt(ml) + (int)wave_mbcnt(mh);
-		const uint32_t idx = (uint32_t)(j * 128 + 2 * lane) << 16;
-		if (vl) s_tok[pl] = idx | vl;
-		if (vh) s_tok[pl + (vl != 0u)] = (idx + 0x10000u) | vh;
-		ntok += __popcll(ml) + __popcll(mh);
-	}
-	CFHD_WAVE_SYNC();
-	ent_count_tokens(seg, job, frame, ntok, lane, s_tok, segs, tables, peak_flags, tokens, probe);
-}
-
-__device__ __forceinline__ void ent_count_tokens(int seg, const EntSegJob &job, int frame, int ntok, int lane, uint32_t *s_tok, EntSegState *segs, const EntTables *tables,
-                                                 uint32_t *peak_flags, uint32_t *tokens, int probe)
-{
-	const EntTables *T = tables + job.table;
-	uint32_t bits = 0, lead32 = 0, lead_valid = 0;
-	if (CFHD_PROBE(probe) == 2) { const unsigned long long q = __ballot(s_tok[lane] == 0x12345u); if (lane == 0) { EntSegState &z = segs[seg]; z.first_nz = -1; z.last_nz = -1; z.bits = q == 0x123456789ull && ntok == 0x12345; z.ntok = 0; z.lead32 = 0; z.lead_valid = 0; } return; }
-	uint32_t npeaks = 0;
-	for (int t0 = 0; t0 < ntok; t0 += ENT_LANES) {
+struct EntTokCarry { int ntok, first_idx, last_idx; uint32_t bits, npeaks, lead32, lead_valid; };
+__device__ __forceinline__ EntTokCarry ent_tok_carry() { EntTokCarry c; c.ntok = 0; c.first_idx = -1; c.last_idx = -1; c.bits = 0; c.npeaks = 0; c.lead32 = 0; c.lead_valid = 0; return c; }
+
+__device__ __forceinline__ void ent_count_window(const EntSegJob &job, const EntTables *T, int nwin, int lane, const uint32_t *s_tok, uint32_t *seg_out, EntTokCarry &c, int probe)
+{
+	for (int t0 = 0; t0 < nwin; t0 += ENT_LANES) {
 		const int t = t0 + lane;
-		const bool have = t < ntok;
+		const bool have = t < nwin;
 		const uint32_t tok = have ? s_tok[t] : 0u;
-		const uint32_t before = (have && t > 0) ? s_tok[t - 1] : 0u;
-		const uint32_t run = (have && t > 0) ? (tok >> 16) - (before >> 16) - 1u : 0u;
+		const bool follows = have && (t > 0 || c.ntok > 0);
+		const uint32_t before = follows ? (t > 0 ? s_tok[t - 1] >> 16 : (uint32_t)c.last_idx) : 0u;
+		const uint32_t run = follows ? (tok >> 16) - before - 1u : 0u;
+		const bool long_run = run >= 3072u;
+		const uint32_t ri = long_run ? 0u : run;
 		int value = (int)(int16_t)(tok & 0xffffu);
 		const bool is_peak = job.table && (value > ENT_PEAK_THRESHOLD || value < -ENT_PEAK_THRESHOLD);
 		if (is_peak) value = value > 0 ? ENT_PEAK_THRESHOLD + 1 : -ENT_PEAK_THRESHOLD - 1;
-		npeaks += (uint32_t)__popcll(__ballot(is_peak));
+		c.npeaks += (uint32_t)__popcll(__ballot(is_peak));
 		const uint32_t ve = value_entry(T, value);
-		const uint32_t rt = T->run_total[run];
-		const uint2 rp = T->run_pack[run];
+		uint32_t rt = T->run_total[ri];
+		if (__ballot(long_run)) { if (long_run) rt = run_bits_any(T, run); }
+		const uint2 rp = T->run_pack[ri];
 		uint32_t my_top = 0, my_len = 0;
 		if (have) {
-			bits += rt + (ve >> 27);
-			uint32_t *seg_out = tokens + (size_t)seg * ENT_TOK_STRIDE;
+			c.bits += rt + (ve >> 27);
 			const uint32_t vs = ve >> 27, vc = ve & 0x7FFFFFFu, rs = run ? rp.y & 0xffu : 0u;
-			const bool simple = (run == 0u || (rp.y >> 8) == run) && rs + vs <= (uint32_t)ENT_STR_BITS;
+			const bool simple = !long_run && (run == 0u || (rp.y >> 8) == run) && rs + vs <= (uint32_t)ENT_STR_BITS;
 			const uint32_t str = simple ? (((run ? rp.x : 0u) << vs) | vc) << (32u - rs - vs) : 0u;
 			const uint32_t len = simple ? rs + vs : (uint32_t)ENT_CODE_COMPLEX;
-			const uint32_t rec = simple ? str | len : (run << 22) | (((uint32_t)value & 0xffffu) << 6) | len;
-			if (CFHD_PROBE(probe) != 4) seg_out[t] = rec;
+			const int v11 = value < -1023 ? -1023 : (value > 1023 ? 1023 : value);
+			const uint32_t rec = simple ? str | len : (run << ENT_REC_RUN_SHIFT) | (((uint32_t)v11 & 0x7ffu) << 6) | len;
+			if (CFHD_PROBE(probe) != 4) seg_out[c.ntok + t] = rec;
 			my_top = str; my_len = len;
 		}
-		if (t0 == 0) {
-			const int hi = ntok < ENT_LANES ? ntok : ENT_LANES;
+		if (t0 == 0 && c.ntok == 0) {
+			const int hi = nwin < ENT_LANES ? nwin : ENT_LANES;
 			const unsigned long long cx = __ballot(have && my_len == (uint32_t)ENT_CODE_COMPLEX);
 			const uint32_t l = (have && my_len != (uint32_t)ENT_CODE_COMPLEX) ? my_len : 0u;
 			const uint32_t sc = wave_incl_scan(l), ex = sc - l;
@@ -230,24 +219,62 @@
 			uint32_t part = (lane < stop_lane && ex < 32u) ? my_top >> ex : 0u;
 #pragma unroll
 			for (int d = 1; d < ENT_LANES; d <<= 1) part |= __shfl_xor(part, d);
-			lead32 = part;
+			c.lead32 = part;
 			const uint32_t known = stop_lane > 0 ? wave_get(sc, stop_lane - 1) : 0u;
-			lead_valid = known < 32u ? known : 32u;
-		}
-	}
-	if (npeaks && lane == 0) atomic_or_u32(&peak_flags[frame], 1u);
-	bits = wave_get(wave_incl_scan(bits), ENT_LANES - 1);
+			c.lead_valid = known < 32u ? known : 32u;
+		}
+	}
+	if (nwin) {
+		if (!c.ntok) c.first_idx = (int)(s_tok[0] >> 16);
+		c.last_idx = (int)(s_tok[nwin - 1] >> 16);
+		c.ntok += nwin;
+	}
+}
+
+__device__ __forceinline__ void ent_count_finish(int seg, const EntSegJob &job, int frame, size_t tok_base, int lane, const EntTokCarry &c, EntSegState *segs, uint32_t *peak_flags)
+{
+	if (c.npeaks && lane == 0) atomic_or_u32(&peak_flags[frame], 1u);
+	const uint32_t bits = wave_get(wave_incl_scan(c.bits), ENT_LANES - 1);
 	if (lane == 0) {
 		EntSegState &s = segs[seg];
-		s.first_nz = ntok ? job.first + (int)(s_tok[0] >> 16) : -1;
-		s.last_nz = ntok ? job.first + (int)(s_tok[ntok - 1] >> 16) : -1;
+		s.first_nz = c.ntok ? job.first + c.first_idx : -1;
+		s.last_nz = c.ntok ? job.first + c.last_idx : -1;
 		s.bits = bits;
-		s.ntok = (uint32_t)ntok;
-		s.lead32 = lead32; s.lead_valid = lead_valid;
+		s.ntok = (uint32_t)c.ntok;
+		s.lead32 = c.lead32; s.lead_valid = c.lead_valid;
+		s.tok_blk = (uint32_t)(tok_base / ENT_TOK_STRIDE);
 		s.out = nullptr;
-		s.info = (job.first != 0 ? 1u : 0u) | (job.first + ENT_SEG < job.n ? 2u : 0u) | ((uint32_t)job.table << 8);
-		s.peaks = npeaks;
-	}
+		s.info = (job.first != 0 ? 1u : 0u) | (job.first + job.len < job.n ? 2u : 0u) | ((uint32_t)job.table << 8);
+		s.peaks = c.npeaks;
+	}
+}
+
+__device__ __forceinline__ void ent_count_segment(int seg, const EntSegJob &job, int frame, size_t tok_base, uint32_t *w, int lane, uint32_t *s_tok, EntSegState *segs, const EntTables *tables,
+                                                  uint32_t *peak_flags, uint32_t *tokens, int probe)
+{
+	if (CFHD_PROBE(probe) == 1) { uint32_t o = 0; for (int j = 0; j < ENT_SEG / 128; j++) o |= w[j]; const unsigned long long q = __ballot(o == 0x12345u); if (lane == 0) { EntSegState &z = segs[seg]; z.first_nz = -1; z.last_nz = -1; z.bits = q == 0x123456789ull; z.ntok = 0; z.lead32 = 0; z.lead_valid = 0; } return; }
+	const EntTables *T = tables + job.table;
+	EntTokCarry c = ent_tok_carry();
+	const int span = job.n - job.first < job.len ? job.n - job.first : job.len;
+	for (int off = 0; off < span; off += ENT_SEG) {
+		if (off) ent_load_segment(job, lane, w, off);
+		int nwin = 0;
+#pragma unroll
+		for (int j = 0; j < ENT_SEG / 128; j++) {
+			const uint32_t vl = w[j] & 0xffffu, vh = w[j] >> 16;
+			const unsigned long long ml = __ballot(vl != 0u), mh = __ballot(vh != 0u);
+			const int pl = nwin + (int)wave_mbcnt(ml) + (int)wave_mbcnt(mh);
+			const uint32_t idx = (uint32_t)(off + j * 128 + 2 * lane) << 16;
+			if (vl) s_tok[pl] = idx | vl;
+			if (vh) s_tok[pl + (vl != 0u)] = (idx + 0x10000u) | vh;
+			nwin += __popcll(ml) + __popcll(mh);
+		}
+		CFHD_WAVE_SYNC();
+		if (CFHD_PROBE(probe) == 2) { const unsigned long long q = __ballot(s_tok[lane] == 0x12345u); if (lane == 0) { EntSegState &z = segs[seg]; z.first_nz = -1; z.last_nz = -1; z.bits = q == 0x123456789ull && nwin == 0x12345; z.ntok = 0; z.lead32 = 0; z.lead_valid = 0; } return; }
+		ent_count_window(job, T, nwin, lane, s_tok, tokens + tok_base, c, probe);
+		CFHD_WAVE_SYNC();
+	}
+	ent_count_finish(seg, job, frame, tok_base, lane, c, segs, peak_flags);
 }
 
 enum { ENT_COUNT_SEGS = 1 };
@@ -262,15 +289,15 @@
 	if (idx0 >= total_segs) return;
 	const int seg0 = (idx0 / range_n) * geom.segs_per_frame + range_lo + idx0 % range_n;
 	static_assert(ENT_COUNT_SEGS == 1, "the range mapping takes one segment per wave");
-	EntSegJob job[ENT_COUNT_SEGS]; int frame[ENT_COUNT_SEGS];
+	EntSegJob job[ENT_COUNT_SEGS]; int frame[ENT_COUNT_SEGS]; size_t tok_base[ENT_COUNT_SEGS];
 	uint32_t w[ENT_COUNT_SEGS][ENT_SEG / 128];
 #pragma unroll
 	for (int k = 0; k < ENT_COUNT_SEGS; k++)
-		if (idx0 + k < total_segs) { job[k] = ent_seg_job(seg_jobs, geom, seg0 + k, &frame[k]); ent_load_segment(job[k], lane, w[k]); }
+		if (idx0 + k < total_segs) { job[k] = ent_seg_job(seg_jobs, geom, seg0 + k, &frame[k], &tok_base[k]); ent_load_segment(job[k], lane, w[k]); }
 #pragma unroll
 	for (int k = 0; k < ENT_COUNT_SEGS; k++)
 		if (idx0 + k < total_segs) {
-			ent_count_segment(seg0 + k, job[k], frame[k], w[k], lane, s_tok_all[wave], segs, tables, peak_flags, tokens, probe);
+			ent_count_segment(seg0 + k, job[k], frame[k], tok_base[k], w[k], lane, s_tok_all[wave], segs, tables, peak_flags, tokens, probe);
 			CFHD_WAVE_SYNC();
 		}
 }
@@ -280,61 +307,90 @@
                                                                    uint32_t *peak_flags, uint32_t *tokens, int range_lo, int range_n, EntBlockLists lists)
 {
 	__shared__ uint32_t s_tok_all[ENT_WAVES][ENT_SEG];
+	enum { SPAN_BLOCKS = ENT_BLK_SPAN / 8, HMAX = SPAN_BLOCKS / ENT_LANES };
 	const int lane = wave_lane();
 	const int wave = wave_uniform((int)(threadIdx.x >> 6));
 	const int idx0 = wave_uniform((int)blockIdx.x * ENT_WAVES + wave);
 	if (idx0 >= total_segs) return;
 	const int seg = (idx0 / range_n) * geom.segs_per_frame + range_lo + idx0 % range_n;
-	int frame;
-	const EntSegJob job = ent_seg_job(seg_jobs, geom, seg, &frame);
-	uint32_t *s_tok = s_tok_all[wave];
+	int frame; size_t tok_base;
+	const EntSegJob job = ent_seg_job(seg_jobs, geom, seg, &frame, &tok_base);
+	const EntTables *T = tables + job.table;
+	uint32_t *s_tok = s_tok_all[wave], *seg_out = tokens + tok_base;
 	const int pitch = job.pitch, cpr = (pitch + FWD_CHUNK_COLS_ENT - 1) / FWD_CHUNK_COLS_ENT;
-	const int end = job.first + ENT_SEG < job.n ? job.first + ENT_SEG : job.n;
-	const uint4 *blocks = wave_uniform_ptr(lists.blocks + (size_t)(job.coeffs - lists.coeff0) / 8);
+	const int seg_end = job.first + job.len, end = seg_end < job.n ? seg_end : job.n;
+	const uint4 *band_blocks = lists.blocks + (size_t)(job.coeffs - lists.coeff0) / 8;
 	const unsigned long long *masks = wave_uniform_ptr(lists.masks + (size_t)frame * lists.masks_per_frame + job.mask_base);
-	const int row0 = job.first / pitch, col0 = job.first - row0 * pitch;
-	uint32_t entry[2]; bool listed[2];
-#pragma unroll
-	for (int h = 0; h < 2; h++) {
-		const int q = lane + 64 * h, pos = job.first + 8 * q;
-		int row = row0, col = col0 + 8 * q;
+	EntTokCarry c = ent_tok_carry();
+	for (int s0 = job.first; s0 < end; s0 += ENT_BLK_SPAN) {
+		const int nq = (seg_end - s0 < ENT_BLK_SPAN ? seg_end - s0 : ENT_BLK_SPAN) / 8;
+		const int row0 = s0 / pitch, col0 = s0 - row0 * pitch;
+		const uint4 *blocks = wave_uniform_ptr(band_blocks + (size_t)row0 * (size_t)(pitch >> 3));
+		uint32_t entry[HMAX]; bool listed[HMAX];
+		int row = 0, col = col0 + 8 * lane;
 		while (col >= pitch) { col -= pitch; row++; }
-		static_assert(FWD_CHUNK_COLS_ENT == 62 * 8, "the division below is by 62 blocks");
-		const uint32_t c8 = (uint32_t)col >> 3, k = mul_u24(c8, 1058u) >> 16, i = c8 - mul_u24(k, 62u);
-		unsigned long long m = 0ull;
-		if (pos < end) m = masks[mul_u24((uint32_t)row, (uint32_t)cpr) + k];
-		listed[h] = ((m >> i) & 1ull) != 0ull;
-		entry[h] = ((mul_u24((uint32_t)row, (uint32_t)pitch >> 3) + mul_u24(k, 62u) + (uint32_t)__popcll(m & ((1ull << i) - 1ull))) << 7) | (uint32_t)q;
-	}
-	const unsigned long long b0 = __ballot(listed[0]), b1 = __ballot(listed[1]);
-	const int n0 = __popcll(b0), nlisted = n0 + __popcll(b1);
-	if (listed[0]) s_tok[wave_mbcnt(b0)] = entry[0];
-	if (listed[1]) s_tok[n0 + (int)wave_mbcnt(b1)] = entry[1];
-	CFHD_WAVE_SYNC();
-	const uint32_t mine[2] = { lane < nlisted ? s_tok[lane] : 0u, lane + 64 < nlisted ? s_tok[lane + 64] : 0u };
-	CFHD_WAVE_SYNC();
-	int ntok = 0;
-#pragma unroll
-	for (int h = 0; h < 2; h++) {
-		if (64 * h >= nlisted) break;
-		uint32_t w[4] = { 0u, 0u, 0u, 0u };
-		if (lane + 64 * h < nlisted) { const cfhd_u4 v = CFHD_LDG128(&blocks[mine[h] >> 7]); w[0] = v.x; w[1] = v.y; w[2] = v.z; w[3] = v.w; }
-		uint32_t cnt = 0;
-#pragma unroll
-		for (int d = 0; d < 4; d++) cnt += ((w[d] & 0xffffu) != 0u) + ((w[d] >> 16) != 0u);
-		const uint32_t incl = wave_incl_scan(cnt);
-		uint32_t p = (uint32_t)ntok + incl - cnt;
-		const uint32_t local = 8u * (mine[h] & 127u);
-#pragma unroll
-		for (int d = 0; d < 4; d++) {
-			const uint32_t vl = w[d] & 0xffffu, vh = w[d] >> 16;
-			if (vl) s_tok[p++] = ((local + 2u * d) << 16) | vl;
-			if (vh) s_tok[p++] = ((local + 2u * d + 1u) << 16) | vh;
-		}
-		ntok += (int)wave_get(incl, ENT_LANES - 1);
-	}
-	CFHD_WAVE_SYNC();
-	ent_count_tokens(seg, job, frame, ntok, lane, s_tok, segs, tables, peak_flags, tokens, 0);
+#pragma unroll
+		for (int h = 0; h < HMAX; h++) {
+			listed[h] = false; entry[h] = 0u;
+			if (ENT_LANES * h >= nq) continue;
+			if (h) { col += 8 * ENT_LANES; while (col >= pitch) { col -= pitch; row++; } }
+			const int q = lane + ENT_LANES * h, pos = s0 + 8 * q;
+			static_assert(FWD_CHUNK_COLS_ENT == 62 * 8, "the division below is by 62 blocks");
+			const uint32_t c8 = (uint32_t)col >> 3, k = mul_u24(c8, 1058u) >> 16, i = c8 - mul_u24(k, 62u);
+			unsigned long long m = 0ull;
+			if (pos < end) m = masks[mul_u24((uint32_t)(row0 + row), (uint32_t)cpr) + k];
+			listed[h] = ((m >> i) & 1ull) != 0ull;
+			entry[h] = ((mul_u24((uint32_t)row, (uint32_t)pitch >> 3) + mul_u24(k, 62u) + (uint32_t)__popcll(m & ((1ull << i) - 1ull))) << 9) | (uint32_t)q;
+		}
+		int nlisted = 0;
+#pragma unroll
+		for (int h = 0; h < HMAX; h++) {
+			if (ENT_LANES * h >= nq) break;
+			const unsigned long long b = __ballot(listed[h]);
+			if (listed[h]) s_tok[nlisted + (int)wave_mbcnt(b)] = entry[h];
+			nlisted += __popcll(b);
+		}
+		CFHD_WAVE_SYNC();
+		uint32_t mine[HMAX];
+#pragma unroll
+		for (int h = 0; h < HMAX; h++) mine[h] = lane + ENT_LANES * h < nlisted ? s_tok[lane + ENT_LANES * h] : 0u;
+		CFHD_WAVE_SYNC();
+		int nwin = 0;
+		cfhd_u4 next = { 0u, 0u, 0u, 0u };
+		if (lane < nlisted) next = CFHD_LDG128(&blocks[mine[0] >> 9]);
+#pragma unroll
+		for (int h = 0; h < HMAX; h++) {
+			if (ENT_LANES * h >= nlisted) break;
+			const uint32_t w[4] = { next.x, next.y, next.z, next.w };
+			if (h + 1 < HMAX) {
+				next.x = next.y = next.z = next.w = 0u;
+				if (lane + ENT_LANES * (h + 1) < nlisted) next = CFHD_LDG128(&blocks[mine[h + 1 < HMAX ? h + 1 : h] >> 9]);
+			}
+			uint32_t cnt = 0;
+#pragma unroll
+			for (int d = 0; d < 4; d++) cnt += ((w[d] & 0xffffu) != 0u) + ((w[d] >> 16) != 0u);
+			const uint32_t incl = wave_incl_scan(cnt), total = wave_get(incl, ENT_LANES - 1);
+			if (nwin + (int)total > ENT_SEG) {
+				CFHD_WAVE_SYNC();
+				ent_count_window(job, T, nwin, lane, s_tok, seg_out, c, 0);
+				CFHD_WAVE_SYNC();
+				nwin = 0;
+			}
+			uint32_t p = (uint32_t)nwin + incl - cnt;
+			const uint32_t local = (uint32_t)(s0 - job.first) + 8u * (mine[h] & 511u);
+#pragma unroll
+			for (int d = 0; d < 4; d++) {
+				const uint32_t vl = w[d] & 0xffffu, vh = w[d] >> 16;
+				if (vl) s_tok[p++] = ((local + 2u * d) << 16) | vl;
+				if (vh) s_tok[p++] = ((local + 2u * d + 1u) << 16) | vh;
+			}
+			nwin += (int)total;
+		}
+		CFHD_WAVE_SYNC();
+		ent_count_window(job, T, nwin, lane, s_tok, seg_out, c, 0);
+		CFHD_WAVE_SYNC();
+	}
+	ent_count_finish(seg, job, frame, tok_base, lane, c, segs, peak_flags);
 }
 
 __global__ void __launch_bounds__(ENT_THREADS) k_ent_scan(const EntBandJob *bands, EntSegState *segs, EntBandState *band_state, const EntTables *tables)
@@ -632,9 +688,9 @@
 		uint32_t run = 0, ve = 0;
 		if (__ballot(complex)) {
 			if (complex) {
-				run = rec >> 22;
-				ve = value_entry(T, (int)(int16_t)((rec >> 6) & 0xffffu));
-				len = (uint32_t)T->run_total[run] + (ve >> 27);
+				run = rec >> ENT_REC_RUN_SHIFT;
+				ve = value_entry(T, (int)(rec << (32 - ENT_REC_RUN_SHIFT)) >> 21);
+				len = run_bits_any(T, run) + (ve >> 27);
 			}
 		}
 		const uint32_t sc = wave_incl_scan(len);
@@ -644,7 +700,7 @@
 		if (complex) {
 			uint32_t left = run;
 			while (left > 0u) {
-				const uint2 rc = T->run_pack[left];
+				const uint2 rc = T->run_pack[left < 3072u ? left : 3071u];
 				const uint32_t size = rc.y & 0xffu;
 				ent_put_string(s_words, out, use_lds, first_word, pos, (uint64_t)rc.x << (64u - size));
 				pos += size; left -= rc.y >> 8;
@@ -681,11 +737,6 @@
 	uint32_t first_rec[ENT_EMIT_SEGS];
 	EntSegState st[ENT_EMIT_SEGS + 2];
 #pragma unroll
-	for (int k = 0; k < ENT_EMIT_SEGS; k++) {
-		const int sg = seg0 + k < total_segs ? seg0 + k : seg0;
-		first_rec[k] = tokens[(size_t)sg * ENT_TOK_STRIDE + lane];
-	}
-#pragma unroll
 	for (int k = 0; k < ENT_EMIT_SEGS + 2; k++) {
 		int sg = seg0 - 1 + k;
 		sg = sg < 0 ? 0 : (sg < total_segs ? sg : total_segs - 1);
@@ -693,8 +744,11 @@
 	}
 #pragma unroll
 	for (int k = 0; k < ENT_EMIT_SEGS; k++)
+		first_rec[k] = tokens[(size_t)st[k + 1].tok_blk * ENT_TOK_STRIDE + lane];
+#pragma unroll
+	for (int k = 0; k < ENT_EMIT_SEGS; k++)
 		if (seg0 + k < total_segs) {
-			ent_emit_segment(st[k + 1], st[k], st[k + 2], first_rec[k], tokens + (size_t)(seg0 + k) * ENT_TOK_STRIDE, lane, s_words_all[wave], tables, probe);
+			ent_emit_segment(st[k + 1], st[k], st[k + 2], first_rec[k], tokens + (size_t)st[k + 1].tok_blk * ENT_TOK_STRIDE, lane, s_words_all[wave], tables, probe);
 			CFHD_WAVE_SYNC();
 		}
 }
```
